# jewettaij/visfd

Hardware: AMD Instinct MI355X
Metric: Mvoxels/s (Gauss+DoG+TV pipeline) on 1024^3 float32; % HBM roofline (higher is better)
Workload: dtype f32

## Files before the change

include/visfd_hip.h:

```cpp
#ifndef VISFD_HIP_H
#define VISFD_HIP_H

#include <stddef.h>
#include <stdint.h>

#ifdef __cplusplus
extern "C" {
#endif

#define VISFD_HIP_OK 0
#define VISFD_HIP_EINVAL 1
#define VISFD_HIP_EDEVICE 2
#define VISFD_HIP_ENOMEM 3
#define VISFD_HIP_ECAPACITY 4

#define VISFD_HIP_INCREASING_EIVALS 0
#define VISFD_HIP_DECREASING_EIVALS 1

typedef struct visfd_hip_ctx visfd_hip_ctx;

int visfd_hip_create(int device, void* stream, visfd_hip_ctx** out);
int visfd_hip_destroy(visfd_hip_ctx* ctx);
int visfd_hip_synchronize(visfd_hip_ctx* ctx);
void* visfd_hip_get_stream(visfd_hip_ctx* ctx);
// ... 503 lines not shown
                                   int64_t nvox, int round, uint32_t prefix,
                                   uint64_t* hist_host , uint64_t* n_unmasked_host);
int visfd_hip_select_histogram_todev(visfd_hip_ctx*, const float* saliency, const float* mask, int64_t nvox, int round,
                                     uint32_t prefix, uint64_t* hist_dev );
int visfd_hip_apply_threshold_dev(visfd_hip_ctx*, float* saliency, int64_t nvox, float threshold);

int visfd_hip_tv_dense_stick(visfd_hip_ctx*, const float* saliency, const float* direction,
                             float* tensor, const float* mask_src, const float* mask_dst,
                             int64_t nx, int64_t ny, int64_t nz, float sigma_tv, int exponent,
                             float cutoff_ratio, int detect_curves);
int visfd_hip_tv_dense_stick_dev(visfd_hip_ctx*, const float* saliency, const float* direction,
                                 float* tensor, const float* mask_src, const float* mask_dst,
                                 int64_t nx, int64_t ny, int64_t nz, float sigma_tv, int exponent,
                                 float cutoff_ratio, int detect_curves);
int visfd_hip_tv_dense_stick_slab_dev(visfd_hip_ctx*, const float* saliency, const float* direction,
                                      float* tensor, const float* mask_src, const float* mask_dst,
                                      int64_t nx, int64_t ny, int64_t nz_local, int64_t z_out0,
                                      int64_t z_out1, float sigma_tv, int exponent,
                                      float cutoff_ratio, int detect_curves);
int visfd_hip_tv_weight_sum(visfd_hip_ctx*, const float* saliency, float* den, const float* mask_src, const float* mask_dst,
                            int64_t nx, int64_t ny, int64_t nz, float sigma_tv, float cutoff_ratio);
int visfd_hip_tv_tables(float sigma_tv, float cutoff_ratio, int* halfwidth_out, float* w,
                        float* rhat);

int visfd_hip_tensor_saliency(visfd_hip_ctx*, const float* tensor, const float* mask, int64_t nvox,
                              int eival_order, float* saliency_inout);
int visfd_hip_tensor_saliency_dev(visfd_hip_ctx*, const float* tensor, const float* mask,
                                  int64_t nvox, int eival_order, float* saliency_inout);
int visfd_hip_tensor_saliency_bg_dev(visfd_hip_ctx*, const float* tensor, const float* mask, int64_t nvox, int eival_order,
                                     const float* image, const float* background, float* saliency_inout);

int visfd_hip_membrane_detect(visfd_hip_ctx*, const float* src, const float* mask,
                              int64_t nx, int64_t ny, int64_t nz, float sigma, float truncate_ratio,
                              int eival_order, float best_fraction, float threshold_abs, float sigma_tv,
                              int tv_exponent, float tv_cutoff_ratio, float* saliency_out,
                              float* tensor_out, float* direction_out, float* threshold_out);
int visfd_hip_membrane_detect_dev(visfd_hip_ctx*, const float* src, const float* mask,
                                  int64_t nx, int64_t ny, int64_t nz, float sigma, float truncate_ratio,
                                  int eival_order, float best_fraction, float threshold_abs,
                                  float sigma_tv, int tv_exponent, float tv_cutoff_ratio,
                                  float* saliency_out, float* tensor_out, float* direction_out,
                                  float* threshold_out);
int visfd_hip_membrane_detect_bg(visfd_hip_ctx*, const float* src, const float* mask,
                                 int64_t nx, int64_t ny, int64_t nz, float sigma, float truncate_ratio,
                                 int eival_order, float best_fraction, float threshold_abs, float sigma_tv,
                                 int tv_exponent, float tv_cutoff_ratio, float sigma_background, int normalize_background,
                                 float* saliency_out, float* tensor_out, float* direction_out, float* threshold_out);
int visfd_hip_membrane_detect_bg_dev(visfd_hip_ctx*, const float* src, const float* mask,
                                     int64_t nx, int64_t ny, int64_t nz, float sigma, float truncate_ratio,
                                     int eival_order, float best_fraction, float threshold_abs,
                                     float sigma_tv, int tv_exponent, float tv_cutoff_ratio, float sigma_background,
                                     int normalize_background, float* saliency_out, float* tensor_out, float* direction_out,
                                     float* threshold_out);

int visfd_hip_apply_gauss_slab_dev(visfd_hip_ctx*, const float* src, float* dst,
                                   int64_t nx, int64_t ny, int64_t nz_local, int64_t z_lo,
                                   int64_t nz_global, const float sigma[3], const int halfwidth[3],
                                   int normalize, float* A_out);

typedef struct visfd_hip_slab visfd_hip_slab;
typedef struct visfd_hip_transport {
  int (*sendrecv)(void* user, int peer, const void* sendbuf, void* recvbuf, size_t bytes, void* stream);
  int (*allreduce_sum_u64)(void* user, uint64_t* buf, size_t count, void* stream);
  int (*group_start)(void* user);
  int (*group_end)(void* user);
  void* user;
} visfd_hip_transport;
int visfd_hip_slab_unique_id(void* id_out_128_bytes);
int visfd_hip_slab_rccl_available(void);
int visfd_hip_slab_create_rccl(visfd_hip_ctx*, const void* unique_id_128_bytes , int rank,
                               int world, int64_t nz_global, int ghost, visfd_hip_slab** out);
int visfd_hip_slab_create_custom(visfd_hip_ctx*, const visfd_hip_transport*, int rank, int world, int64_t nz_global,
                                 int ghost, visfd_hip_slab** out);
int visfd_hip_slab_destroy(visfd_hip_slab*);
int visfd_hip_slab_layout(visfd_hip_slab*, int64_t out[7]);
int visfd_hip_slab_selftest(visfd_hip_slab*, int64_t count);
int visfd_hip_slab_set_reserve(visfd_hip_slab*, int reserve_workgroups);
int visfd_hip_slab_exchange_dev(visfd_hip_slab*, float* const* volumes, int nvol, int64_t nx, int64_t ny, int depth);
int visfd_hip_membrane_detect_slab_dev(visfd_hip_slab*, float* src, float* sal, float* dirs, float* tensor, float* scratch,
                                       int64_t nx, int64_t ny, float sigma, float truncate_ratio, int eival_order,
                                       float best_fraction, float sigma_tv, int exponent, float tv_truncate_ratio,
                                       int src_halo_ready, float* threshold_out);
int visfd_hip_membrane_detect_slab(visfd_hip_slab*, const float* src_owned, int64_t nx, int64_t ny, float sigma,
                                   float truncate_ratio, int eival_order, float best_fraction, float sigma_tv, int exponent,
                                   float tv_truncate_ratio, float* sal_owned, float* tensor_owned, float* threshold_out);
int visfd_hip_membrane_detect_slab_bg_dev(visfd_hip_slab*, float* src, float* sal, float* dirs, float* tensor, float* scratch,
                                          float* background, int64_t nx, int64_t ny, float sigma, float truncate_ratio,
                                          int eival_order, float best_fraction, float sigma_tv, int exponent,
                                          float tv_truncate_ratio, float sigma_background, int normalize_background,
                                          int src_halo_ready, float* threshold_out);
int visfd_hip_membrane_detect_slab_bg(visfd_hip_slab*, const float* src_owned, int64_t nx, int64_t ny, float sigma,
                                      float truncate_ratio, int eival_order, float best_fraction, float sigma_tv, int exponent,
                                      float tv_truncate_ratio, float sigma_background, int normalize_background,
                                      float* sal_owned, float* tensor_owned, float* threshold_out);
int visfd_hip_blob_dog_slab_dev(visfd_hip_slab*, float* src, int64_t nx, int64_t ny, const float* blob_sigma, int n_sigma,
                                float delta_sigma_over_sigma, float truncate_ratio, float minima_threshold,
                                float maxima_threshold, int src_halo_ready,
                                visfd_hip_blob* minima, int64_t minima_capacity, int64_t* n_minima,
                                visfd_hip_blob* maxima, int64_t maxima_capacity, int64_t* n_maxima);
int visfd_hip_blob_halo_depth(const float* blob_sigma, int n_sigma, float delta_sigma_over_sigma, float truncate_ratio,
                              int* depth_out);
int visfd_hip_apply_gauss_slab(visfd_hip_slab*, const float* src_owned, int64_t nx, int64_t ny, const float sigma[3],
                               const int halfwidth[3], int normalize, float* dst_owned, float* A_out);
int visfd_hip_blob_dog_slab(visfd_hip_slab*, const float* src_owned, int64_t nx, int64_t ny, const float* blob_sigma, int n_sigma,
                            float delta_sigma_over_sigma, float truncate_ratio, float minima_threshold, float maxima_threshold,
                            visfd_hip_blob* minima, int64_t minima_capacity, int64_t* n_minima,
// ... 39 lines not shown
```

visfd_amd/api.py:

```python
import ctypes as C
import os
import sys

import numpy as np

_HERE = os.path.dirname(os.path.abspath(__file__))
LIB_PATH = os.environ.get("VISFD_HIP_LIB") or os.path.join(_HERE, "libvisfd_hip.so")

INCREASING_EIVALS = 0
DECREASING_EIVALS = 1

MORPH_DILATE, MORPH_ERODE, MORPH_OPEN, MORPH_CLOSE, MORPH_TOP_HAT_WHITE, MORPH_TOP_HAT_BLACK = range(6)
MORPH_PATH_GENERAL, MORPH_PATH_XRUNS, MORPH_PATH_LEVELS = 0, 1, 2
MEDIAN_PATH_GENERAL, MEDIAN_PATH_TILED = 0, 1
FILTER3D_PATH_GENERAL, FILTER3D_PATH_TILED = 0, 1
DISTANCE_PATH_GENERAL, DISTANCE_PATH_TRANSFORM = 0, 1
DISTANCE_MAX_DIM_SUM = 46340

_fp = C.POINTER(C.c_float)
_ip = C.POINTER(C.c_int)
_i64 = C.c_int64
_vp = C.c_void_p


# ... 150 lines not shown
                                     C.c_float, C.c_float, C.c_int, C.POINTER(Blob), _i64, C.POINTER(_i64),
                                     C.POINTER(Blob), _i64, C.POINTER(_i64)]),
    "visfd_hip_blob_dog_dev": (C.c_int, [_vp, _vp, _vp, _i64, _i64, _i64, _fp, C.c_int, _fp, C.c_float, C.c_float,
                                         C.c_float, C.c_float, C.c_int, C.POINTER(Blob), _i64, C.POINTER(_i64),
                                         C.POINTER(Blob), _i64, C.POINTER(_i64)]),
    "visfd_hip_blob_dog_begin_dev": (C.c_int, [_vp, _vp, _vp, _i64, _i64, _i64, _fp, C.c_int, _fp, C.c_float, C.c_float,
                                               C.c_float, C.c_float, C.c_int, C.POINTER(_vp)]),
    "visfd_hip_blob_dog_end": (C.c_int, [_vp, C.POINTER(Blob), _i64, C.POINTER(_i64), C.POINTER(Blob), _i64, C.POINTER(_i64)]),
    "visfd_hip_blob_dog_abort": (None, [_vp]),
    "visfd_hip_blob_jobs_pending": (C.c_int, [_vp]),
    "visfd_hip_debug_poison_workspace": (C.c_int, [_vp]),
    "visfd_hip_blob_diameters_to_sigmas": (C.c_int, [_fp, C.c_int, _fp]),
    "visfd_hip_blob_sigmas_to_diameters": (C.c_int, [_fp, C.c_int, _fp]),
    "visfd_hip_calc_hessian": (C.c_int, [_vp, _vp, _vp, _vp, _vp, _i64, _i64, _i64, C.c_float, C.c_float]),
    "visfd_hip_calc_hessian_dev": (C.c_int, [_vp, _vp, _vp, _vp, _vp, _i64, _i64, _i64, C.c_float, C.c_float]),
    "visfd_hip_diagonalize_flat_sym3": (C.c_int, [_vp, _vp, _vp, _i64, C.c_int]),
    "visfd_hip_diagonalize_flat_sym3_dev": (C.c_int, [_vp, _vp, _vp, _i64, C.c_int]),
    "visfd_hip_hessian_saliency": (C.c_int, [_vp, _vp, _vp, _i64, C.c_int, _vp, _vp]),
    "visfd_hip_hessian_saliency_dev": (C.c_int, [_vp, _vp, _vp, _i64, C.c_int, _vp, _vp]),
    "visfd_hip_ridge_saliency_dev": (C.c_int, [_vp, _vp, _vp, _i64, _i64, _i64, C.c_float, C.c_float, C.c_int,
                                               _vp, _vp]),
    "visfd_hip_ridge_scores_dev": (C.c_int, [_vp, _vp, _vp, _i64, _i64, _i64, C.c_float, C.c_float, C.c_int, _vp, _vp]),
    "visfd_hip_ridge_directions_dev": (C.c_int, [_vp, _vp, _i64, _i64, _i64, C.c_float, C.c_int, _vp, _vp]),
    "visfd_hip_threshold_fraction": (C.c_int, [_vp, _vp, _vp, _i64, C.c_float, _fp]),
    "visfd_hip_threshold_fraction_dev": (C.c_int, [_vp, _vp, _vp, _i64, C.c_float, _fp]),
    "visfd_hip_select_histogram_dev": (C.c_int, [_vp, _vp, _vp, _i64, C.c_int, C.c_uint32,
                                                 C.POINTER(C.c_uint64), C.POINTER(C.c_uint64)]),
    "visfd_hip_select_histogram_todev": (C.c_int, [_vp, _vp, _vp, _i64, C.c_int, C.c_uint32, _vp]),
    "visfd_hip_get_stream": (_vp, [_vp]),
    "visfd_hip_apply_threshold_dev": (C.c_int, [_vp, _vp, _i64, C.c_float]),
    "visfd_hip_tv_dense_stick": (C.c_int, [_vp, _vp, _vp, _vp, _vp, _vp, _i64, _i64, _i64, C.c_float, C.c_int,
                                           C.c_float, C.c_int]),
    "visfd_hip_tv_dense_stick_dev": (C.c_int, [_vp, _vp, _vp, _vp, _vp, _vp, _i64, _i64, _i64, C.c_float, C.c_int,
                                               C.c_float, C.c_int]),
    "visfd_hip_tv_dense_stick_slab_dev": (C.c_int, [_vp, _vp, _vp, _vp, _vp, _vp, _i64, _i64, _i64, _i64, _i64,
                                                    C.c_float, C.c_int, C.c_float, C.c_int]),
    "visfd_hip_tv_tables": (C.c_int, [C.c_float, C.c_float, _ip, _fp, _fp]),
    "visfd_hip_tv_weight_sum": (C.c_int, [_vp, _vp, _vp, _vp, _vp, _i64, _i64, _i64, C.c_float, C.c_float]),
    "visfd_hip_membrane_detect": (C.c_int, [_vp, _vp, _vp, _i64, _i64, _i64, C.c_float, C.c_float, C.c_int, C.c_float,
                                            C.c_float, C.c_float, C.c_int, C.c_float, _vp, _vp, _vp, _fp]),
    "visfd_hip_membrane_detect_dev": (C.c_int, [_vp, _vp, _vp, _i64, _i64, _i64, C.c_float, C.c_float, C.c_int,
                                                C.c_float, C.c_float, C.c_float, C.c_int, C.c_float, _vp, _vp, _vp,
                                                _fp]),
    "visfd_hip_tensor_saliency": (C.c_int, [_vp, _vp, _vp, _i64, C.c_int, _vp]),
    "visfd_hip_tensor_saliency_dev": (C.c_int, [_vp, _vp, _vp, _i64, C.c_int, _vp]),
    "visfd_hip_peak_background_dev": (C.c_int, [_vp, _vp, _vp, _i64, _i64, _i64, C.c_float, C.c_float, C.c_int, _vp]),
    "visfd_hip_ridge_scores_bg_dev": (C.c_int, [_vp, _vp, _vp, _i64, _i64, _i64, C.c_float, C.c_float, C.c_int, _vp, _vp, _vp]),
    "visfd_hip_tensor_saliency_bg_dev": (C.c_int, [_vp, _vp, _vp, _i64, C.c_int, _vp, _vp, _vp]),
    "visfd_hip_membrane_detect_bg": (C.c_int, [_vp, _vp, _vp, _i64, _i64, _i64, C.c_float, C.c_float, C.c_int, C.c_float,
                                               C.c_float, C.c_float, C.c_int, C.c_float, C.c_float, C.c_int, _vp, _vp, _vp, _fp]),
    "visfd_hip_membrane_detect_bg_dev": (C.c_int, [_vp, _vp, _vp, _i64, _i64, _i64, C.c_float, C.c_float, C.c_int,
                                                   C.c_float, C.c_float, C.c_float, C.c_int, C.c_float, C.c_float, C.c_int,
                                                   _vp, _vp, _vp, _fp]),
    "visfd_hip_membrane_detect_slab_bg_dev": (C.c_int, [_vp, _vp, _vp, _vp, _vp, _vp, _vp, _i64, _i64, C.c_float, C.c_float, C.c_int,
                                                        C.c_float, C.c_float, C.c_int, C.c_float, C.c_float, C.c_int, C.c_int, _fp]),
    "visfd_hip_membrane_detect_slab_bg": (C.c_int, [_vp, _vp, _i64, _i64, C.c_float, C.c_float, C.c_int, C.c_float, C.c_float,
                                                    C.c_int, C.c_float, C.c_float, C.c_int, _vp, _vp, _fp]),
    "visfd_hip_bin_array3d": (C.c_int, [_vp, _vp, C.POINTER(_i64), _vp, C.POINTER(_i64), _ip]),
    "visfd_hip_bin_array3d_dev": (C.c_int, [_vp, _vp, C.POINTER(_i64), _vp, C.POINTER(_i64), _ip]),
    "visfd_hip_unbin_array3d": (C.c_int, [_vp, _vp, C.POINTER(_i64), _vp, C.POINTER(_i64), _ip]),
    "visfd_hip_unbin_array3d_dev": (C.c_int, [_vp, _vp, C.POINTER(_i64), _vp, C.POINTER(_i64), _ip]),
    "visfd_hip_label_connected": (C.c_int, [_vp, _vp, _vp, _i64, _i64, _i64, C.c_float, _vp, C.c_float, C.c_float, C.c_int,
                                            _vp, C.c_float, C.c_float, C.c_int, C.c_int, _i64, C.c_int, C.c_int, C.c_int,
                                            C.POINTER(_i64), _vp, _vp, _vp, _i64]),
    "visfd_hip_label_connected_ex": (C.c_int, [_vp, _vp, _vp, _i64, _i64, _i64, C.c_float, _vp, C.c_float, C.c_float, C.c_int,
                                               _vp, C.c_float, C.c_float, C.c_int, C.c_int, _i64, C.c_int, C.c_int, C.c_int,
                                               C.POINTER(_i64), _vp, _vp, _vp, _i64, _vp, _vp, _vp, _i64, _vp]),
    "visfd_hip_label_connected_device_seeds": (C.c_int, [_vp, _vp, _vp, _vp, _i64, _i64, _i64, C.c_float, _vp, C.c_float,
                                                         C.c_float, C.c_int, _vp, C.c_float, C.c_float, C.c_int, C.c_int, _i64,
                                                         C.c_int, C.c_int, C.c_int, C.POINTER(_i64), _vp, _vp, _vp, _i64, _vp,
                                                         _vp, _vp, _i64, _vp]),
    "visfd_hip_label_connected_device_seeds_last": (C.c_int, [_vp, _ip, C.POINTER(_i64)]),
    "visfd_hip_label_connected_graph": (C.c_int, [_vp] + _LABEL_CONNECTED_EX),
    "visfd_hip_label_connected_graph_dev": (C.c_int, [_vp] + _LABEL_CONNECTED_EX),
    "visfd_hip_label_connected_graph_host": (C.c_int, list(_LABEL_CONNECTED_EX)),
    "visfd_hip_label_connected_graph_last": (C.c_int, [_vp, _ip, C.POINTER(C.c_uint), C.POINTER(_i64), C.POINTER(_i64)]),
    "visfd_hip_label_connected_graph_last_times": (C.c_int, [_vp, _fp]),
    "visfd_hip_label_connected_graph_last_settled": (C.c_int, [_vp, C.POINTER(C.c_uint)]),
    "visfd_hip_principal_directions_host": (C.c_int, [_vp, _vp, _i64, C.c_int, _vp]),
    "visfd_hip_tensor_saliency_host": (C.c_int, [_vp, _vp, _i64, C.c_int, _vp]),
    "visfd_hip_diagonalize_sym3_f32_host": (C.c_int, [_vp, C.c_int, _vp, _vp]),
    "visfd_hip_diagonalize_flat_sym3_host": (C.c_int, [_vp, _vp, _i64, C.c_int]),
    "visfd_hip_convert_flat_sym2_evects3_host": (C.c_int, [_vp, C.c_int, _vp, _vp]),
    "visfd_hip_surface_points": (C.c_int, [_vp, _vp, _vp, _vp, _i64, _i64, _i64, C.c_int, _fp, C.c_float, C.c_int, C.c_float,
                                           _vp, _vp, _i64, C.POINTER(_i64)]),
    "visfd_hip_surface_points_ctx": (C.c_int, [_vp, _vp, _vp, _vp, _vp, _i64, _i64, _i64, C.c_int, _fp, C.c_float, C.c_int,
                                               C.c_float, _vp, _vp, _i64, C.POINTER(_i64)]),
    "visfd_hip_surface_points_dev": (C.c_int, [_vp, _vp, _vp, _vp, _vp, _i64, _i64, _i64, C.c_int, _fp, C.c_float, C.c_int,
                                               C.c_float, _vp, _vp, _i64, C.POINTER(_i64)]),
    "visfd_hip_surface_points_last": (C.c_int, [_vp, C.POINTER(_i64)]),
    "visfd_hip_surface_points_last_times": (C.c_int, [_vp, _fp]),
    "visfd_hip_sphere_overlap": (C.c_float, [C.c_float, C.c_float, C.c_float]),
    "visfd_hip_sort_blobs": (C.c_int, [_fp, _fp, _fp, _i64, C.c_int, C.c_int, C.POINTER(C.c_uint64)]),
    "visfd_hip_discard_masked_blobs": (C.c_int, [_fp, _fp, _fp, C.POINTER(_i64), _vp, _i64, _i64, _i64]),
    "visfd_hip_discard_overlapping_blobs": (C.c_int, [_fp, _fp, _fp, C.POINTER(_i64), C.c_float, C.c_float,
                                                     C.c_float, C.c_int, C.c_int]),
    "visfd_hip_discard_overlapping_blobs_ctx": (C.c_int, [_vp, _vp, _vp, _vp, C.POINTER(_i64), C.c_float, C.c_float,
                                                         C.c_float, C.c_int, C.c_int]),
    "visfd_hip_discard_overlapping_blobs_dev": (C.c_int, [_vp, _vp, _vp, _vp, C.POINTER(_i64), C.c_float, C.c_float,
                                                         C.c_float, C.c_int, C.c_int]),
    "visfd_hip_discard_overlapping_blobs_last": (C.c_int, [_vp, C.POINTER(_i64)]),
    "visfd_hip_discard_overlapping_blobs_last_times": (C.c_int, [_vp, _fp]),
    "visfd_hip_voxelize_mesh": (C.c_int, _VOXELIZE),
    "visfd_hip_voxelize_mesh_dev": (C.c_int, _VOXELIZE),
    "visfd_hip_voxelize_last": (C.c_int, [_vp, C.POINTER(_i64)]),
    "visfd_hip_voxelize_last_times": (C.c_int, [_vp, _fp]),
# ... 1582 lines not shown
    def dilate_dev(self, src, dst, dxyz, b, mask=None):
        self.morph_table_dev(MORPH_DILATE, src, dst, dxyz, b, mask)

    def erode_dev(self, src, dst, dxyz, b, mask=None):
        self.morph_table_dev(MORPH_ERODE, src, dst, dxyz, b, mask)

    def gauss_slab_dev(self, src, dst, z_lo, nz_global, sigma, hw, normalize=True):
        nz, ny, nx = src.shape
        A = C.c_float()
        self._chk(self._L.visfd_hip_apply_gauss_slab_dev(self._h, _dev(src), _dev(dst), nx, ny, nz, int(z_lo),
                                                         int(nz_global), _f3(sigma), _i3(hw), int(normalize),
                                                         C.byref(A)))
        return A.value

    def log_dev(self, src, dst, sigma, delta, ratio, mask=None):
        nz, ny, nx = src.shape
        self._chk(self._L.visfd_hip_apply_log_dev(self._h, _dev(src), _dev(dst), _dev(mask), nx, ny, nz,
                                                  _f3(sigma), float(delta), float(ratio), None, None))

    def blob_dog_dev(self, src, sigmas, mask=None, aspect=None, delta=0.02, ratio=2.5, minima_threshold=np.inf,
                     maxima_threshold=-np.inf, use_ratios=False, cap=1 << 16):
        return self._blob_call(self._L.visfd_hip_blob_dog_dev, _dev(src), _dev(mask), tuple(src.shape), sigmas,
                               aspect, delta, ratio, minima_threshold, maxima_threshold, use_ratios, cap)

    def calc_hessian_dev(self, src, grad, hess, sigma, ratio, mask=None):
        nz, ny, nx = src.shape
        self._chk(self._L.visfd_hip_calc_hessian_dev(self._h, _dev(src), _dev(grad), _dev(hess), _dev(mask), nx,
                                                     ny, nz, float(sigma), float(ratio)))

    def hessian_saliency_dev(self, hess, sal, dirs, order, mask=None):
        self._chk(self._L.visfd_hip_hessian_saliency_dev(self._h, _dev(hess), _dev(mask), sal.numel(), int(order),
                                                         _dev(sal), _dev(dirs)))

    def ridge_saliency_dev(self, src, sal, dirs, sigma, ratio, order, mask=None):
        nz, ny, nx = src.shape
        self._chk(self._L.visfd_hip_ridge_saliency_dev(self._h, _dev(src), _dev(mask), nx, ny, nz, float(sigma),
                                                       float(ratio), int(order), _dev(sal), _dev(dirs)))

    def ridge_scores_dev(self, src, sal, smoothed, sigma, ratio, order, mask=None, background=None):
        nz, ny, nx = src.shape
        self._chk(self._L.visfd_hip_ridge_scores_bg_dev(self._h, _dev(src), _dev(mask), nx, ny, nz, float(sigma),
                                                        float(ratio), int(order), _dev(background), _dev(sal), _dev(smoothed)))

    def peak_background_dev(self, src, background, sigma_background, ratio, mask=None, normalize=True):
        nz, ny, nx = src.shape
        self._chk(self._L.visfd_hip_peak_background_dev(self._h, _dev(src), _dev(mask), nx, ny, nz, float(sigma_background),
                                                        float(ratio), int(bool(normalize)), _dev(background)))

    def ridge_directions_dev(self, smoothed, sal, dirs, sigma, order):
        nz, ny, nx = smoothed.shape
        self._chk(self._L.visfd_hip_ridge_directions_dev(self._h, _dev(smoothed), nx, ny, nz, float(sigma), int(order),
                                                         _dev(sal), _dev(dirs)))

    def threshold_fraction_dev(self, sal, fraction, mask=None):
        thr = C.c_float()
        self._chk(self._L.visfd_hip_threshold_fraction_dev(self._h, _dev(sal), _dev(mask), sal.numel(),
                                                           float(fraction), C.byref(thr)))
        return thr.value

    def select_histogram_dev(self, sal, pass_, prefix, mask=None):
        hist = np.zeros(2048, np.uint64)
        n = C.c_uint64()
        self._chk(self._L.visfd_hip_select_histogram_dev(self._h, _dev(sal), _dev(mask), sal.numel(), int(pass_),
                                                         int(prefix), hist.ctypes.data_as(C.POINTER(C.c_uint64)),
                                                         C.byref(n)))
        return hist, int(n.value)

    def select_histogram_todev(self, sal, pass_, prefix, hist, mask=None):
        assert hist.is_cuda and hist.numel() == 2048 and hist.element_size() == 8 and hist.is_contiguous()
        self._chk(self._L.visfd_hip_select_histogram_todev(self._h, _dev(sal), _dev(mask), sal.numel(), int(pass_),
                                                           int(prefix), hist.data_ptr()))

    def stream_handle(self):
        return int(self._L.visfd_hip_get_stream(self._h) or 0)

    def apply_threshold_dev(self, sal, thr):
        self._chk(self._L.visfd_hip_apply_threshold_dev(self._h, _dev(sal), sal.numel(), float(thr)))

    def tv_dense_stick_dev(self, sal, dirs, tensor, sigma_tv, exponent=4, cutoff=2.0 ** 0.5, mask_src=None,
                           mask_dst=None, curves=False, z_out=None):
        nz, ny, nx = sal.shape
        z0, z1 = (0, nz) if z_out is None else z_out
        self._chk(self._L.visfd_hip_tv_dense_stick_slab_dev(self._h, _dev(sal), _dev(dirs), _dev(tensor),
                                                            _dev(mask_src), _dev(mask_dst), nx, ny, nz, int(z0),
                                                            int(z1), float(sigma_tv), int(exponent), float(cutoff),
                                                            int(curves)))

    def tensor_saliency_dev(self, tensor, sal, order, mask=None, image=None, background=None):
        self._chk(self._L.visfd_hip_tensor_saliency_bg_dev(self._h, _dev(tensor), _dev(mask), sal.numel(), int(order),
                                                           _dev(image), _dev(background), _dev(sal)))


class Slab:

    def __init__(self, ctx, rank, world, nz_global, ghost, transport="rccl", group=None):
        import torch
        import torch.distributed as dist
        self.ctx, self.rank, self.world = ctx, int(rank), int(world)
        self._L = load_library()
        self._h = _vp()
        self._keep = None
        if transport == "rccl_loopback":
            assert world == 1
            idbuf = (C.c_char * 128)()
            ctx._chk(self._L.visfd_hip_slab_unique_id(C.addressof(idbuf)))
            ctx._chk(self._L.visfd_hip_slab_create_rccl(ctx._h, C.addressof(idbuf), 0, 1, nz_global, ghost, C.byref(self._h)))
# ... 192 lines not shown
```

visfd_amd/build.py:

```python
import concurrent.futures
import os
import subprocess
import sys
import time

HERE = os.path.dirname(os.path.abspath(__file__))
ROOT = os.path.dirname(HERE)
CSRC = os.path.join(HERE, "csrc")
OBJDIR = os.path.join(ROOT, "build", "visfd_hip")
LIB = os.path.join(HERE, "libvisfd_hip.so")

SOURCES = ["host_math.cpp", "blob_post.cpp", "connect.cpp", "watershed_host.cpp", "context.hip", "api.hip", "blob_job.hip", "gauss.hip", "blob.hip", "select.hip", "tv.hip", "resample.hip", "slab.hip", "morph.hip", "morph_levels.hip", "extrema.hip", "filter3d.hip", "draw.hip", "watershed.hip", "median.hip", "intensity.hip", "distance.hip", "find_spheres.hip", "discard_overlap.hip", "connect_seeds.hip", "connect_graph_host.cpp", "connect_graph.hip", "voxelize.hip", "surface_points.hip", "close_surface.hip"]
TV_VARIANT = [("tv_tiled.hip", "tv_tiled", ["-fno-slp-vectorize"]), ("tv_box.hip", "tv_box", ["-fno-slp-vectorize"]),
              ("tv_list.hip", "tv_list", ["-fno-slp-vectorize"]),
              ("ridge.hip", "ridge", [])]
PAIR_FLAGS = ["-fno-slp-vectorize"]
VARIANTS = TV_VARIANT + [("gauss_pair.hip", "gauss_pair", PAIR_FLAGS)] + [("gauss_fused.hip", "gauss_fused_h%d" % h, ["-DVH_FUSED_H=%d" % h, "-fno-slp-vectorize"])
                         for h in range(1, 9)]
HEADERS = ["common.hpp", "exact_div.hpp", "tv_common.hpp", "eigen3.hpp", "union_find.hpp", "tile.hpp", "watershed_host.hpp", "intensity.hpp", "connect_host.hpp", "connect_graph.hpp", os.path.join("..", "..", "include", "visfd_hip.h")]

HIPCC = os.environ.get("HIPCC", "/opt/rocm/bin/hipcc")
FLAGS = ["--offload-arch=gfx950", "-O3", "-std=c++17", "-fPIC", "-ffp-contract=off", "-fno-fast-math",
         "-Wall", "-Wno-unused-function"]


def _mtime(p):
    return os.path.getmtime(p) if os.path.exists(p) else 0.0


def _compile(src, obj, extra=()):
    t0 = time.time()
    cmd = [HIPCC] + FLAGS + list(extra) + ["-x", "hip", "-c", os.path.join(CSRC, src), "-o", obj]
    r = subprocess.run(cmd, capture_output=True, text=True)
    return src, r.returncode, r.stdout + r.stderr, time.time() - t0


def build(force=False, jobs=4, verbose=True):
    os.makedirs(OBJDIR, exist_ok=True)
    newest_header = max(_mtime(os.path.join(CSRC, h)) for h in HEADERS)
    todo, objs = [], []
    units = [(s, os.path.splitext(s)[0], []) for s in SOURCES] + VARIANTS
    flagfile = os.path.join(OBJDIR, "flags.txt")
    flagsig = repr((FLAGS, VARIANTS))
    if not os.path.exists(flagfile) or open(flagfile).read() != flagsig:
        force = True
    for s, stem, extra in units:
        obj = os.path.join(OBJDIR, stem + ".o")
        objs.append(obj)
        if force or _mtime(obj) < max(_mtime(os.path.join(CSRC, s)), newest_header):
            todo.append((s, obj, extra))
    if todo:
        with concurrent.futures.ThreadPoolExecutor(max_workers=jobs) as ex:
            for (src, rc, out, dt), (_, obj, _e) in zip(ex.map(lambda a: _compile(*a), todo), todo):
                if verbose:
                    print("[visfd_amd.build] %-22s %5.1fs %s" % (os.path.basename(obj), dt, "ok" if rc == 0 else "FAILED"))
                if rc != 0:
                    sys.stderr.write(out)
                    raise RuntimeError("hipcc failed on " + src)
                elif out.strip() and verbose:
                    sys.stderr.write(out)
    with open(flagfile, "w") as f:
        f.write(flagsig)
    if todo or not os.path.exists(LIB) or _mtime(LIB) < max(_mtime(o) for o in objs):
        cmd = [HIPCC, "--offload-arch=gfx950", "-shared", "-fPIC", "-o", LIB] + objs
        r = subprocess.run(cmd, capture_output=True, text=True)
        if r.returncode != 0:
            sys.stderr.write(r.stdout + r.stderr)
            raise RuntimeError("link failed")
        if verbose:
            print("[visfd_amd.build] linked", LIB)
    build_cli(verbose)
    return LIB
# ... 28 lines not shown
```

visfd_amd/csrc/api.hip:

```cpp
#include <algorithm>
#include <cmath>
#include <vector>

#include "common.hpp"

namespace vh {

int gauss_dev(visfd_hip_ctx* ctx, const float* src, float* dst, const float* mask, i64 nx, i64 ny, i64 nz,
              const float sigma[3], const int hw[3], bool normalize, const GaussOpts& o) {
  VH_REQUIRE(ctx && src && dst && sigma && hw, "null argument");
  std::vector<float> t[3];
  for (int d = 0; d < 3; d++) {
    VH_REQUIRE(sigma[d] >= 0.0f, "sigma must be non-negative");
    VH_REQUIRE(hw[d] >= 0 && hw[d] <= MAX_HALFWIDTH, "filter halfwidth must be in [0, 64]");
    t[d].resize(2 * hw[d] + 1);
    host_gauss_taps(sigma[d], hw[d], t[d].data());
  }
  return dev_separable3d(ctx, src, dst, mask, nx, ny, nz, t[0].data(), hw[0], t[1].data(), hw[1], t[2].data(), hw[2],
                         normalize, o);
}

static int log_pair_try(visfd_hip_ctx* ctx, const float* src, float* dst, i64 nx, i64 ny, i64 nz, const float sa[3],
                        const float sb[3], const int hw[3], float scale, float* A, float* B) {
  if (!ctx || !src || !dst || !sa || !sb || !hw || ctx->opt.log_pair == 0) return GAUSS_DECLINED;
  LogPairRequest rq = {};
  rq.src = src; rq.dst = dst; rq.nx = nx; rq.ny = ny; rq.nz = nz; rq.scale = scale;
  for (int d = 0; d < 3; d++) {
    if (!(sa[d] >= 0.0f) || !(sb[d] >= 0.0f) || hw[d] < 0 || hw[d] > MAX_HALFWIDTH) return GAUSS_DECLINED;
    rq.a[d].h = rq.b[d].h = hw[d];
    host_gauss_taps(sa[d], hw[d], rq.a[d].t);
    host_gauss_taps(sb[d], hw[d], rq.b[d].t);
  }
  const int rc = log_pair_route(ctx, rq);
  if (rc != VISFD_HIP_OK) return rc;
  if (A) *A = (rq.a[0].t[hw[0]] * rq.a[1].t[hw[1]]) * rq.a[2].t[hw[2]];
  if (B) *B = (rq.b[0].t[hw[0]] * rq.b[1].t[hw[1]]) * rq.b[2].t[hw[2]];
  return VISFD_HIP_OK;
}

static int dog_dev(visfd_hip_ctx* ctx, const float* src, float* dst, const float* mask, i64 nx, i64 ny, i64 nz,
                   const float sa[3], const float sb[3], const int hw[3], float scale, float* A, float* B) {
  if (!mask) {
    const int rc = log_pair_try(ctx, src, dst, nx, ny, nz, sa, sb, hw, scale, A, B);
    if (rc != GAUSS_DECLINED) return rc;
  }
  VH_TRY(gauss_dev(ctx, src, dst, mask, nx, ny, nz, sa, hw, true, {A}));
  return gauss_dev(ctx, src, dst, mask, nx, ny, nz, sb, hw, true, {B, dst, scale});
}

LogPlan plan_log(const float sigma[3], float delta, float ratio) {
  LogPlan p;
  for (int d = 0; d < 3; d++) {
    p.sa[d] = (float)(sigma[d] * (1.0 - 0.5 * delta));
    p.sb[d] = (float)(sigma[d] * (1.0 + 0.5 * delta));
    p.hw[d] = (int)std::floor(ratio * std::fmax(p.sa[d], p.sb[d]));
  }
  p.scale = (float)(1.0 / (delta * delta));
// ... 280 lines not shown
  float *aos, *ph, *dm, *dsal, *pdir;
  VH_TRY(st.up_planar(WS_H2D_0, WS_H2D_2, hess, 6, &ph, &aos));
  VH_TRY(st.up(WS_H2D_1, mask, &dm));
  VH_TRY(st.out(WS_H2D_3, &dsal));
  VH_TRY(st.out(WS_H2D_4, &pdir, 3));
  VH_TRY(dev_hessian_saliency(ctx, ph, dm, nvox, order, dsal, pdir));
  VH_TRY(st.down(sal, dsal));
  return st.down_interleaved(dir, pdir, aos, 3, dm, true);
}

int visfd_hip_ridge_saliency_dev(visfd_hip_ctx* ctx, const float* src, const float* mask, int64_t nx, int64_t ny,
                                 int64_t nz, float sigma, float ratio, int order, float* sal, float* dir) {
  VH_REQUIRE(ctx && src && sal && dir, "null argument");
  VH_REQUIRE(order == 0 || order == 1, "unsupported eigenvalue order");
  VH_HIP(hipSetDevice(ctx->device));
  VH_TRY(check_dims(nx, ny, nz));
  float* S = nullptr;
  VH_TRY(gauss_iso_dev(ctx, src, nullptr, mask, nx, ny, nz, sigma, ratio, true, "filter halfwidth", &S));
  return dev_ridge_saliency_fused(ctx, S, mask, nx, ny, nz, sigma, order, sal, dir);
}

int visfd_hip_ridge_scores_bg_dev(visfd_hip_ctx* ctx, const float* src, const float* mask, int64_t nx, int64_t ny,
                                  int64_t nz, float sigma, float ratio, int order, const float* background, float* sal,
                                  float* smoothed) {
  VH_REQUIRE(ctx && src && sal && smoothed, "null argument");
  VH_REQUIRE(smoothed != src && smoothed != sal, "the smoothed volume needs its own buffer");
  VH_REQUIRE(order == 0 || order == 1, "unsupported eigenvalue order");
  VH_HIP(hipSetDevice(ctx->device));
  VH_TRY(check_dims(nx, ny, nz));
  VH_TRY(gauss_iso_dev(ctx, src, smoothed, mask, nx, ny, nz, sigma, ratio, true, "filter halfwidth"));
  return dev_ridge_score(ctx, smoothed, mask, nx, ny, nz, sigma, order, sal, background ? src : nullptr, background);
}
int visfd_hip_ridge_scores_dev(visfd_hip_ctx* ctx, const float* src, const float* mask, int64_t nx, int64_t ny,
                               int64_t nz, float sigma, float ratio, int order, float* sal, float* smoothed) {
  return visfd_hip_ridge_scores_bg_dev(ctx, src, mask, nx, ny, nz, sigma, ratio, order, nullptr, sal, smoothed);
}
int visfd_hip_peak_background_dev(visfd_hip_ctx* ctx, const float* src, const float* mask, int64_t nx, int64_t ny,
                                  int64_t nz, float sigma_background, float ratio, int normalize, float* background) {
  VH_REQUIRE(ctx && src && background && background != src, "bad argument");
  VH_REQUIRE(sigma_background > 0.0f, "the background width must be positive");
  VH_HIP(hipSetDevice(ctx->device));
  VH_TRY(check_dims(nx, ny, nz));
  return gauss_iso_dev(ctx, src, background, mask, nx, ny, nz, sigma_background, ratio, normalize != 0,
                       "background filter halfwidth");
}

int visfd_hip_ridge_directions_dev(visfd_hip_ctx* ctx, const float* smoothed, int64_t nx, int64_t ny, int64_t nz,
                                   float sigma, int order, const float* sal, float* dir) {
  VH_REQUIRE(ctx && smoothed && sal && dir, "null argument");
  VH_REQUIRE(order == 0 || order == 1, "unsupported eigenvalue order");
  VH_HIP(hipSetDevice(ctx->device));
  VH_TRY(check_dims(nx, ny, nz));
  return dev_ridge_directions(ctx, smoothed, sal, nx, ny, nz, sigma, order, dir);
}

int visfd_hip_threshold_fraction_dev(visfd_hip_ctx* ctx, float* sal, const float* mask, int64_t nvox,
                                     float fraction, float* thr_out) {
  VH_REQUIRE(ctx && sal && nvox > 0, "bad argument");
  VH_REQUIRE(fraction >= 0.0f && fraction <= 1.0f, "fraction must be in [0,1]");
  VH_HIP(hipSetDevice(ctx->device));
  return dev_threshold_fraction(ctx, sal, mask, nvox, fraction, thr_out);
}

int visfd_hip_threshold_fraction(visfd_hip_ctx* ctx, float* sal, const float* mask, int64_t nvox, float fraction,
                                 float* thr_out) {
  VH_REQUIRE(ctx && sal && nvox > 0, "bad argument");
  VH_REQUIRE(fraction >= 0.0f && fraction <= 1.0f, "fraction must be in [0,1]");
  VH_HIP(hipSetDevice(ctx->device));
  const Stage st = {ctx, (size_t)nvox};
  float *ds, *dm;
  VH_TRY(st.up(WS_H2D_0, sal, &ds));
  VH_TRY(st.up(WS_H2D_1, mask, &dm));
  VH_TRY(dev_threshold_fraction(ctx, ds, dm, nvox, fraction, thr_out));
  return st.down(sal, ds);
}

int visfd_hip_select_histogram_dev(visfd_hip_ctx* ctx, const float* sal, const float* mask, int64_t nvox,
                                   int pass, uint32_t prefix, uint64_t* hist_host, uint64_t* n_unmasked) {
  VH_REQUIRE(ctx && sal && hist_host && nvox > 0, "bad argument");
  VH_REQUIRE(pass >= 0 && pass <= 2, "round must be 0, 1 or 2");
  VH_HIP(hipSetDevice(ctx->device));
  return dev_select_histogram(ctx, sal, mask, nvox, pass, prefix, hist_host, n_unmasked);
}

int visfd_hip_select_histogram_todev(visfd_hip_ctx* ctx, const float* sal, const float* mask, int64_t nvox, int pass,
                                     uint32_t prefix, uint64_t* hist_dev) {
  VH_REQUIRE(ctx && sal && hist_dev && nvox > 0, "bad argument");
  VH_REQUIRE(pass >= 0 && pass <= 2, "round must be 0, 1 or 2");
  VH_HIP(hipSetDevice(ctx->device));
  return dev_select_histogram_todev(ctx, sal, mask, nvox, pass, prefix, hist_dev);
}

int visfd_hip_apply_threshold_dev(visfd_hip_ctx* ctx, float* sal, int64_t nvox, float thr) {
  VH_REQUIRE(ctx && sal && nvox > 0, "bad argument");
  VH_HIP(hipSetDevice(ctx->device));
  return dev_apply_threshold(ctx, sal, nvox, thr);
}

int visfd_hip_bin_array3d_dev(visfd_hip_ctx* ctx, const float* src, const int64_t size_src[3], float* dst,
                              const int64_t size_dst[3], const int* offset) {
  VH_REQUIRE(ctx && src && dst && size_src && size_dst, "null argument");
  VH_HIP(hipSetDevice(ctx->device));
  return dev_bin_array3d(ctx, src, size_src, dst, size_dst, offset);
}

int visfd_hip_unbin_array3d_dev(visfd_hip_ctx* ctx, const float* src, const int64_t size_src[3], float* dst,
// ... 37 lines not shown

int visfd_hip_tv_dense_stick_slab_dev(visfd_hip_ctx* ctx, const float* sal, const float* dir, float* ten,
                                      const float* mask_src, const float* mask_dst, int64_t nx,
                                      int64_t ny, int64_t nz_local, int64_t z_out0, int64_t z_out1,
                                      float sigma_tv, int exponent, float cutoff, int curves) {
  VH_REQUIRE(ctx && sal && dir && ten, "null argument");
  VH_HIP(hipSetDevice(ctx->device));
  return dev_tv_dense_stick(ctx, sal, dir, ten, mask_src, mask_dst, nx, ny, nz_local, z_out0, z_out1,
                            sigma_tv, exponent, cutoff, curves != 0);
}

int visfd_hip_tv_dense_stick_dev(visfd_hip_ctx* ctx, const float* sal, const float* dir, float* ten,
                                 const float* mask_src, const float* mask_dst, int64_t nx, int64_t ny,
                                 int64_t nz, float sigma_tv, int exponent, float cutoff, int curves) {
  return visfd_hip_tv_dense_stick_slab_dev(ctx, sal, dir, ten, mask_src, mask_dst, nx, ny, nz, 0, nz,
                                           sigma_tv, exponent, cutoff, curves);
}

int visfd_hip_tv_dense_stick(visfd_hip_ctx* ctx, const float* sal, const float* dir, float* ten, const float* mask_src,
                             const float* mask_dst, int64_t nx, int64_t ny, int64_t nz, float sigma_tv, int exponent,
                             float cutoff, int curves) {
  VH_REQUIRE(ctx && sal && dir && ten, "null argument");
  VH_HIP(hipSetDevice(ctx->device));
  VH_TRY(check_dims(nx, ny, nz));
  const Stage st = {ctx, (size_t)(nx * ny * nz)};
  float *dsal, *pdir, *pten, *aos6, *dms = nullptr, *dmd = nullptr;
  VH_TRY(st.up(WS_H2D_0, sal, &dsal));
  VH_TRY(st.up_planar(WS_H2D_1, WS_H2D_2, dir, 3, &pdir));
  VH_TRY(st.out(WS_H2D_3, &pten, 6));
  VH_TRY(st.up(WS_H2D_4, mask_src, &dms));
  if (mask_dst == mask_src) dmd = dms;
  else VH_TRY(st.up(WS_A, mask_dst, &dmd));
  VH_TRY(dev_tv_dense_stick(ctx, dsal, pdir, pten, dms, dmd, nx, ny, nz, 0, nz, sigma_tv, exponent, cutoff, curves != 0));
  VH_TRY(st.out(WS_B, &aos6, 6));
  return st.down_interleaved(ten, pten, aos6, 6, dmd, true);
}

int visfd_hip_tv_weight_sum(visfd_hip_ctx* ctx, const float* sal, float* den, const float* mask_src,
                            const float* mask_dst, int64_t nx, int64_t ny, int64_t nz, float sigma_tv, float cutoff) {
  VH_REQUIRE(ctx && sal && den, "null argument");
  VH_HIP(hipSetDevice(ctx->device));
  VH_TRY(check_dims(nx, ny, nz));
  const Stage st = {ctx, (size_t)(nx * ny * nz)};
  float *dsal, *dden, *dms = nullptr, *dmd = nullptr;
  VH_TRY(st.up(WS_H2D_0, sal, &dsal));
  VH_TRY(st.up(WS_H2D_1, den, &dden));
  VH_TRY(st.up(WS_H2D_4, mask_src, &dms));
  if (mask_dst == mask_src) dmd = dms;
  else VH_TRY(st.up(WS_A, mask_dst, &dmd));
  VH_TRY(dev_tv_weight_sum(ctx, dsal, dden, dms, dmd, nx, ny, nz, sigma_tv, cutoff));
  return st.down(den, dden);
}

int visfd_hip_membrane_detect_bg_dev(visfd_hip_ctx* ctx, const float* src, const float* mask, int64_t nx,
                                     int64_t ny, int64_t nz, float sigma, float ratio, int order,
                                     float best_fraction, float threshold_abs, float sigma_tv, int exponent,
                                     float cutoff, float sigma_background, int normalize_background, float* sal, float* ten,
                                     float* dir, float* thr_out) {
  VH_REQUIRE(ctx && src && sal, "null argument");
  VH_REQUIRE(order == 0 || order == 1, "unsupported eigenvalue order");
  VH_REQUIRE(best_fraction <= 1.0f, "fraction must be <= 1");
  VH_HIP(hipSetDevice(ctx->device));
  VH_TRY(check_dims(nx, ny, nz));
  const i64 n = nx * ny * nz;
  float* d = dir;
  if (!d) VH_TRY(ws(ctx, WS_TVAUX, (size_t)(3 * n), &d));
  float* smoothed = nullptr;
  VH_TRY(ws(ctx, WS_D, (size_t)n, &smoothed));
  float* bg = nullptr;
  if (sigma_background > 0.0f) {
    VH_TRY(ws(ctx, WS_C, (size_t)n, &bg));
    VH_TRY(visfd_hip_peak_background_dev(ctx, src, mask, nx, ny, nz, sigma_background, ratio, normalize_background, bg));
  }
  VH_TRY(visfd_hip_ridge_scores_bg_dev(ctx, src, mask, nx, ny, nz, sigma, ratio, order, bg, sal, smoothed));
  float thr = threshold_abs;
  if (best_fraction >= 0.0f) VH_TRY(dev_threshold_fraction(ctx, sal, mask, n, best_fraction, &thr));
  else VH_TRY(dev_apply_threshold(ctx, sal, n, thr));
  if (thr_out) *thr_out = thr;
  if (dir) VH_HIP(hipMemsetAsync(dir, 0, sizeof(float) * 3 * (size_t)n, ctx->stream));
  VH_TRY(dev_ridge_directions(ctx, smoothed, sal, nx, ny, nz, sigma, order, d));
  if (sigma_tv > 0.0f) {
    float* t = ten;
    if (!t) VH_TRY(ws(ctx, WS_B, (size_t)(6 * n), &t));
    VH_TRY(dev_tv_dense_stick(ctx, sal, d, t, mask, mask, nx, ny, nz, 0, nz, sigma_tv, exponent, cutoff, false));
    VH_TRY(dev_tensor_saliency(ctx, t, mask, n, order, sal, bg ? src : nullptr, bg));
  }
  return VISFD_HIP_OK;
}
int visfd_hip_membrane_detect_dev(visfd_hip_ctx* ctx, const float* src, const float* mask, int64_t nx,
                                  int64_t ny, int64_t nz, float sigma, float ratio, int order,
                                  float best_fraction, float threshold_abs, float sigma_tv, int exponent,
                                  float cutoff, float* sal, float* ten, float* dir, float* thr_out) {
  return visfd_hip_membrane_detect_bg_dev(ctx, src, mask, nx, ny, nz, sigma, ratio, order, best_fraction, threshold_abs, sigma_tv,
                                          exponent, cutoff, 0.0f, 1, sal, ten, dir, thr_out);
}

int visfd_hip_membrane_detect_bg(visfd_hip_ctx* ctx, const float* src, const float* mask, int64_t nx, int64_t ny,
                                 int64_t nz, float sigma, float ratio, int order, float best_fraction,
                                 float threshold_abs, float sigma_tv, int exponent, float cutoff,
                                 float sigma_background, int normalize_background, float* sal, float* ten, float* dir,
                                 float* thr_out) {
  VH_REQUIRE(ctx && src && sal, "null argument");
  VH_HIP(hipSetDevice(ctx->device));
  VH_TRY(check_dims(nx, ny, nz));
  const Stage st = {ctx, (size_t)(nx * ny * nz)};
  float *ds, *dm, *dsal, *pdir, *pten = nullptr, *aos = nullptr;
  VH_TRY(st.up(WS_H2D_0, src, &ds));
  VH_TRY(st.up(WS_H2D_1, mask, &dm));
  VH_TRY(st.out(WS_H2D_2, &dsal));
  VH_TRY(st.out(WS_H2D_3, &pdir, 3));
  if (ten && sigma_tv > 0.0f) {
    VH_TRY(st.out(WS_H2D_4, &pten, 6));
    VH_HIP(hipMemsetAsync(pten, 0, sizeof(float) * 6 * st.n, ctx->stream));
  }
  VH_TRY(visfd_hip_membrane_detect_bg_dev(ctx, ds, dm, nx, ny, nz, sigma, ratio, order, best_fraction, threshold_abs, sigma_tv,
                                          exponent, cutoff, sigma_background, normalize_background, dsal, pten, pdir, thr_out));
  VH_TRY(st.down(sal, dsal));
  if ((ten && pten) || dir) VH_TRY(st.out(WS_A, &aos, 6));
  if (ten && pten) VH_TRY(st.down_interleaved(ten, pten, aos, 6, nullptr, false));
  if (dir) VH_TRY(st.down_interleaved(dir, pdir, aos, 3, nullptr, false));
  return VISFD_HIP_OK;
}
int visfd_hip_membrane_detect(visfd_hip_ctx* ctx, const float* src, const float* mask, int64_t nx, int64_t ny,
                              int64_t nz, float sigma, float ratio, int order, float best_fraction,
                              float threshold_abs, float sigma_tv, int exponent, float cutoff, float* sal,
                              float* ten, float* dir, float* thr_out) {
  return visfd_hip_membrane_detect_bg(ctx, src, mask, nx, ny, nz, sigma, ratio, order, best_fraction, threshold_abs, sigma_tv,
                                      exponent, cutoff, 0.0f, 1, sal, ten, dir, thr_out);
}

int visfd_hip_tensor_saliency_bg_dev(visfd_hip_ctx* ctx, const float* ten, const float* mask, int64_t nvox,
                                     int order, const float* image, const float* background, float* sal) {
  VH_REQUIRE(ctx && ten && sal && nvox > 0, "bad argument");
  VH_REQUIRE((image == nullptr) == (background == nullptr), "image and background come as a pair");
  VH_REQUIRE(order == 0 || order == 1, "unsupported eigenvalue order");
  VH_HIP(hipSetDevice(ctx->device));
  return dev_tensor_saliency(ctx, ten, mask, nvox, order, sal, image, background);
}
int visfd_hip_tensor_saliency_dev(visfd_hip_ctx* ctx, const float* ten, const float* mask, int64_t nvox,
                                  int order, float* sal) {
// ... 175 lines not shown
```

visfd_amd/csrc/common.hpp:

```cpp
#pragma once

#include <hip/hip_runtime.h>

#include <cstdint>
#include <cstdio>
#include <cstring>
#include <string>
#include <vector>

#include "../../include/visfd_hip.h"

namespace vh {

typedef int64_t i64;

void set_error(const std::string& msg);
int fail(int code, const std::string& msg);

#define VH_HIP(expr)                                                                         \
  do {                                                                                       \
    hipError_t _e = (expr);                                                                  \
    if (_e != hipSuccess)                                                                    \
      return vh::fail(_e == hipErrorOutOfMemory ? VISFD_HIP_ENOMEM : VISFD_HIP_EDEVICE,      \
                      std::string(#expr) + ": " + hipGetErrorString(_e));                    \
// ... 20 lines not shown
  WS_HIST,
  WS_TVTAB,
  WS_TVAUX,
  WS_TVSCRATCH,
  WS_TVLIST,
  WS_H2D_0, WS_H2D_1, WS_H2D_2, WS_H2D_3, WS_H2D_4,
  WS_MORPH_TAB,
  WS_MORPH_SRC,
  WS_MORPH_TMP,
  WS_EXT_FLAGS,
  WS_EXT_PARENT,
  WS_EXT_COUNT,
  WS_EXT_COUNTERS,
  WS_EXT_LIST,
  WS_EXT_RANKS,
  WS_F3D_TAB,
  WS_DRAW_OWNER,
  WS_DRAW_TAB,
  WS_WSH_KIND,
  WS_WSH_LINK,
  WS_WSH_C,
  WS_WSH_STATE,
  WS_WSH_SEEDS,
  WS_WSH_FLAGS,
  WS_MEDIAN_TAB,
  WS_INTENSITY,
  WS_DIST_DSQ,
  WS_DIST_STACK,
  WS_DIST_POINTS,
  WS_FS_RECORDS,
  WS_FS_QUERIES,
  WS_CG_WORD,
  WS_CG_AUX,
  WS_CG_LIST,
  WS_CG_REC,
  WS_CG_SEEDS,
  WS_CG_CLUSTER,
  WS_CG_COUNTERS,
  WS_CG_SETTLE,
  WS_CG_LINKS,
  WS_OVL_LIST,
  WS_OVL_CELLS,
  WS_OVL_TEMP,
  WS_VOX_TOGGLE,
  WS_VOX_MESH,
  WS_SP_BITS,
  WS_SP_CHUNKS,
  WS_SP_LIST,
  WS_SP_OUT,
  WS_SP_SCRATCH,
  WS_CS_ACC,
  WS_CS_GRID,
  WS_CS_AUX,
  WS_NSLOTS
};

struct BlobJob;

}

struct visfd_hip_options {
  int gauss_3pass = 0;
  int gauss_cfg = 0;
  int gauss_wg_per_cu = 2;
  int log_pair = 1;
  int log_pair_chunk = 0;
  int tv_dense = 0;
  int tv_fma = 0;
  int gauss_fma = 0;
  int eig_f32 = 0;
  int tv_zrun = 0;
  int tv_no_replay = 0;
  int tv_exact_tiled = 0;
  int tv_no_fold = 0;
  int tv_poison = 0;
  int tv_reserve_wg = 0;
  int tv_max_wg = 0;
  int64_t blob_test_cap = 0;
  int morph_general = 0;
  int morph_levels = 1;
  int filter3d_general = 0;
  int median_general = 0;
  int distance_general = 0;
  int discard_overlap_host = 0;
  int discard_overlap_time = 0;
  int discard_overlap_max_rounds = 256;
  int find_spheres_host = 0;
  int watershed_host = 0;
  int stats_blocks = 0;
  int connect_time = 0;
  int connect_settle = 0;
  int draw_time = 0;
  int voxelize_bisect = 0;
  int voxelize_time = 0;
  int surface_steps_cap = 256;
  int surface_points_time = 0;
  int close_surface_rtol_exp = 5;
  int close_surface_max_cycles = 20;
  int close_surface_time = 0;
  int debug = 0;
};

struct visfd_hip_ctx {
  visfd_hip_options opt;
  int device = 0;
  hipStream_t stream = nullptr;
  bool own_stream = false;
  void* slot_ptr[vh::WS_NSLOTS] = {};
  size_t slot_bytes[vh::WS_NSLOTS] = {};
  std::vector<unsigned char> slot_key[vh::WS_NSLOTS];
  int num_cus = 256;
  hipStream_t aux_stream = nullptr;
  int morph_last_path = -1;
  struct {
    int64_t n = 0, ncols = 0;
    float den = 0.0f;
  } f3d;
  int f3d_last_path = -1;
  int median_last_path = -1;
  int distance_last_path = -1;
  int find_spheres_last_path = -1;
  int64_t discard_overlap_last[8] = {-1, 0, 0, 0, 0, 0, 0, 0};
  float discard_overlap_ms[5] = {-1.0f, -1.0f, -1.0f, -1.0f, -1.0f};
  float draw_ms[3] = {-1.0f, -1.0f, -1.0f};
  int64_t voxelize_stats[4] = {-1, -1, -1, -1};
  float voxelize_ms[3] = {-1.0f, -1.0f, -1.0f};
  int64_t surface_points_last[6] = {-1, 0, -1, -1, -1, -1};
  float surface_points_ms[4] = {-1.0f, -1.0f, -1.0f, -1.0f};
  int64_t close_surface_last[6] = {-1, -1, -1, -1, -1, -1};
  double close_surface_values[2] = {0.0, 0.0};
  float close_surface_ms[3] = {-1.0f, -1.0f, -1.0f};
  int64_t wsh_stats[4] = {-1, -1, -1, -1};
  int64_t connect_seeds[2] = {-1, -1};
  int64_t connect_graph[4] = {-1, 0, -1, -1};
  unsigned connect_graph_settled = 0;
  float connect_graph_ms[8] = {-1.0f, -1.0f, -1.0f, -1.0f, -1.0f, -1.0f, -1.0f, -1.0f};
  std::vector<vh::BlobJob*> blob_jobs;
};

namespace vh {

int blob_jobs_drain(visfd_hip_ctx* ctx, const BlobJob* except = nullptr);
void blob_jobs_abort(visfd_hip_ctx* ctx);

int ws_get(visfd_hip_ctx* ctx, Slot s, size_t bytes, void** out);
template <typename T>
inline int ws(visfd_hip_ctx* ctx, Slot s, size_t count, T** out) {
  void* p = nullptr;
  int rc = ws_get(ctx, s, count * sizeof(T), &p);
  *out = static_cast<T*>(p);
  return rc;
}
bool ws_holds(const visfd_hip_ctx* ctx, Slot s, const void* key, size_t key_bytes);
int ws_put(visfd_hip_ctx* ctx, Slot s, const void* key, size_t key_bytes, const void* host, size_t bytes);

inline int check_dims(i64 nx, i64 ny, i64 nz) {
  if (nx <= 0 || ny <= 0 || nz <= 0) return fail(VISFD_HIP_EINVAL, "image dimensions must be positive");
  return VISFD_HIP_OK;
}
inline bool overlap_bytes(const void* a, size_t na, const void* b, size_t nb) {
  const char* p = static_cast<const char*>(a);
  const char* q = static_cast<const char*>(b);
  return p && q && p < q + nb && q < p + na;
}
inline bool overlaps(const float* a, const float* b, i64 n) { return overlap_bytes(a, sizeof(float) * n, b, sizeof(float) * n); }
// ... 91 lines not shown

constexpr int GAUSS_DECLINED = -1;
int dev_norm_lines(visfd_hip_ctx* ctx, float* D, i64 nx, i64 ny, i64 nz, const Taps& tx, const Taps& ty, const Taps& tz);

struct LogPairRequest {
  const float* src;
  float* dst;
  i64 nx, ny, nz;
  Taps a[3], b[3];
  float scale;
  i64 z_lo, nz_global;
};
int log_pair_route(visfd_hip_ctx* ctx, const LogPairRequest& rq);

int gauss_dev(visfd_hip_ctx* ctx, const float* src, float* dst, const float* mask, i64 nx, i64 ny, i64 nz,
              const float sigma[3], const int hw[3], bool normalize, const GaussOpts& o = {});
struct LogPlan {
  float sa[3], sb[3], scale;
  int hw[3];
};
LogPlan plan_log(const float sigma[3], float delta, float ratio);
int log_dev(visfd_hip_ctx* ctx, const float* src, float* dst, const float* mask, i64 nx, i64 ny, i64 nz,
            const float sigma[3], float delta, float ratio, float* A, float* B);
int dev_sub_square(visfd_hip_ctx* ctx, const float* a, const float* b, float* out, i64 n);
int dev_scale_clamp_sqrt(visfd_hip_ctx* ctx, float* a_inout, i64 n, float scale);

struct ScanPending {
  const unsigned long long* counters = nullptr;
  const void* survivors = nullptr;
  size_t cap_idx = 0, cap_out = 0;
};
int blob_scan_launch(visfd_hip_ctx* ctx, const BlobJob* owner, int set, hipEvent_t done, const float* lo, const float* mid,
                     const float* hi, const float* mask, i64 nx, i64 ny, i64 nz, float min_thr, float max_thr,
                     ScanPending* pending);
int blob_scan_collect(visfd_hip_ctx* ctx, const ScanPending& pending, hipEvent_t done, hipStream_t aux, i64 nx, i64 ny,
                      int scale_index,
                      float sigma, std::vector<visfd_hip_blob>* minima, std::vector<visfd_hip_blob>* maxima,
                      bool* overflow);
int dev_blob_scan(visfd_hip_ctx* ctx, const float* lo, const float* mid, const float* hi,
                  const float* mask, i64 nx, i64 ny, i64 nz, int scale_index, float sigma,
                  float min_thr, float max_thr, bool want_min, bool want_max,
                  std::vector<visfd_hip_blob>* minima, std::vector<visfd_hip_blob>* maxima);

int dev_hessian(visfd_hip_ctx* ctx, const float* smoothed, const float* mask, i64 nx, i64 ny, i64 nz,
                float sigma, float* grad_planar, float* hess_planar);
int dev_hessian_saliency(visfd_hip_ctx* ctx, const float* hess_planar, const float* mask, i64 nvox,
                         int order, float* saliency, float* dir_planar);
int dev_ridge_saliency_fused(visfd_hip_ctx* ctx, const float* smoothed, const float* mask, i64 nx,
                             i64 ny, i64 nz, float sigma, int order, float* saliency,
                             float* dir_planar);
int dev_ridge_score(visfd_hip_ctx* ctx, const float* smoothed, const float* mask, i64 nx, i64 ny, i64 nz,
                    float sigma, int order, float* saliency, const float* peak_img = nullptr, const float* peak_bg = nullptr);
int dev_ridge_directions(visfd_hip_ctx* ctx, const float* smoothed, const float* saliency, i64 nx, i64 ny, i64 nz,
                         float sigma, int order, float* dir_planar);
int dev_diagonalize(visfd_hip_ctx* ctx, const float* m6_planar, float* out6_planar, i64 n, int order);
int dev_tensor_saliency(visfd_hip_ctx* ctx, const float* tensor_planar, const float* mask, i64 nvox,
                        int order, float* saliency, const float* peak_img = nullptr, const float* peak_bg = nullptr);

int dev_select_histogram(visfd_hip_ctx* ctx, const float* sal, const float* mask, i64 nvox, int pass,
                         uint32_t prefix, uint64_t* hist_host, uint64_t* n_unmasked_host);
int dev_select_histogram_todev(visfd_hip_ctx* ctx, const float* sal, const float* mask, i64 nvox, int pass, uint32_t prefix,
                               uint64_t* hist_dev);
int dev_apply_threshold(visfd_hip_ctx* ctx, float* sal, i64 nvox, float thr);
int dev_threshold_fraction(visfd_hip_ctx* ctx, float* sal, const float* mask, i64 nvox, float fraction,
                           float* thr_out);

int dev_tv_dense_stick(visfd_hip_ctx* ctx, const float* sal, const float* dir_planar,
                       float* tensor_planar, const float* mask_src, const float* mask_dst, i64 nx,
                       i64 ny, i64 nz, i64 z_out0, i64 z_out1, float sigma_tv, int exponent,
                       float cutoff, bool curves);

int dev_tv_weight_sum(visfd_hip_ctx* ctx, const float* sal, float* den, const float* mask_src, const float* mask_dst, i64 nx,
                      i64 ny, i64 nz, float sigma_tv, float cutoff);

constexpr int MORPH_RUN_MAX_R = 10;
struct MorphElem {
  i64 n = 0;
  int lo[3] = {0, 0, 0}, hi[3] = {0, 0, 0};
  bool flat = true;
  bool runs = false;
  int R = 0;
  signed char run_len[(2 * MORPH_RUN_MAX_R + 1) * (2 * MORPH_RUN_MAX_R + 1)];
};

int dev_morph_table(visfd_hip_ctx* ctx, const float* src, float* dst, const float* mask, i64 nx, i64 ny, i64 nz,
                    const MorphElem& el, bool dilate, int epi, bool nan_masked, int* path);
int dev_nan_masked(visfd_hip_ctx* ctx, const float* src, const float* mask, float* out, i64 n);
int morph_put_table(visfd_hip_ctx* ctx, const int* dxyz, const float* b, i64 n, MorphElem* el);
int morph_run(visfd_hip_ctx* ctx, const float* src, float* dst, const float* mask, i64 nx, i64 ny, i64 nz, int op,
              MorphElem el);

i64 host_flat_ball_dsq_max(float radius);
constexpr float MORPH_LEVELS_R0 = 5.0f;
int morph_levels_try(visfd_hip_ctx* ctx, const float* src, float* dst, const float* mask, i64 nx, i64 ny, i64 nz, int op,
                     float radius, float radius_max, float bmax, bool* taken);
struct LevelsEpilogue {
  float* dst;
  const float* mask;
  int t;
  unsigned near_bits, far_bits;
  int epi, nan_masked;
};
int dev_distance_levels(visfd_hip_ctx* ctx, const float* src, const float* mask, i64 nx, i64 ny, i64 nz, float level,
                        int32_t* dsq, const LevelsEpilogue& e);

struct MedianTab {
  i64 n = 0;
  int lo[3] = {0, 0, 0}, hi[3] = {0, 0, 0};
  int W = 0, H = 0, D = 0;
};
int median_put_table(visfd_hip_ctx* ctx, const int* dxyz, i64 n, MedianTab* mt);
int median_run(visfd_hip_ctx* ctx, const float* src, float* dst, const float* mask, i64 nx, i64 ny, i64 nz,
               const MedianTab& mt);

int dev_distance_sq(visfd_hip_ctx* ctx, const float* src, const float* mask, i64 nx, i64 ny, i64 nz, float lo, float hi,
// ... 89 lines not shown
```

visfd_amd/csrc/context.hip:

```cpp
#include <cctype>
#include <cstdlib>

#include "common.hpp"

namespace vh {

static thread_local std::string g_last_error;
void set_error(const std::string& msg) { g_last_error = msg; }
int fail(int code, const std::string& msg) {
  g_last_error = msg;
  return code;
}

int ws_get(visfd_hip_ctx* ctx, Slot s, size_t bytes, void** out) {
  if (bytes == 0) bytes = 16;
  if (ctx->slot_bytes[s] < bytes) {
    ctx->slot_key[s].clear();
    if (ctx->slot_ptr[s] && (s == WS_CAND || s == WS_SCANCNT)) VH_TRY(blob_jobs_drain(ctx));
    if (ctx->slot_ptr[s]) {
      VH_HIP(hipStreamSynchronize(ctx->stream));
      VH_HIP(hipFree(ctx->slot_ptr[s]));
      ctx->slot_ptr[s] = nullptr;
      ctx->slot_bytes[s] = 0;
    }
    void* p = nullptr;
    hipError_t e = hipMalloc(&p, bytes);
    if (e != hipSuccess)
      return fail(VISFD_HIP_ENOMEM, "hipMalloc of " + std::to_string(bytes) + " bytes failed: " +
                                        hipGetErrorString(e));
    ctx->slot_ptr[s] = p;
    ctx->slot_bytes[s] = bytes;
  }
  *out = ctx->slot_ptr[s];
  return VISFD_HIP_OK;
}

bool ws_holds(const visfd_hip_ctx* ctx, Slot s, const void* key, size_t key_bytes) {
  const std::vector<unsigned char>& k = ctx->slot_key[s];
  return key_bytes > 0 && k.size() == key_bytes && std::memcmp(k.data(), key, key_bytes) == 0;
}

int ws_put(visfd_hip_ctx* ctx, Slot s, const void* key, size_t key_bytes, const void* host, size_t bytes) {
  ctx->slot_key[s].clear();
  VH_HIP(hipStreamSynchronize(ctx->stream));
  void* d = nullptr;
  VH_TRY(ws_get(ctx, s, bytes, &d));
  VH_HIP(hipMemcpyAsync(d, host, bytes, hipMemcpyHostToDevice, ctx->stream));
  VH_HIP(hipStreamSynchronize(ctx->stream));
  const unsigned char* k = static_cast<const unsigned char*>(key);
  ctx->slot_key[s].assign(k, k + key_bytes);
  return VISFD_HIP_OK;
}

namespace {

struct OptionDesc {
  const char* name;
  int visfd_hip_options::*i = nullptr;
  int64_t visfd_hip_options::*l = nullptr;
  OptionDesc(const char* n, int visfd_hip_options::*f) : name(n), i(f) {}
  OptionDesc(const char* n, int64_t visfd_hip_options::*f) : name(n), l(f) {}
};
#define VH_OPT(field) {#field, &visfd_hip_options::field}
const OptionDesc kOptions[] = {
    VH_OPT(gauss_3pass), VH_OPT(gauss_cfg), VH_OPT(gauss_wg_per_cu), VH_OPT(log_pair), VH_OPT(log_pair_chunk),
    VH_OPT(tv_dense), VH_OPT(tv_fma), VH_OPT(gauss_fma), VH_OPT(eig_f32), VH_OPT(tv_zrun), VH_OPT(tv_no_replay),
    VH_OPT(tv_exact_tiled), VH_OPT(tv_no_fold), VH_OPT(tv_poison), VH_OPT(tv_reserve_wg), VH_OPT(tv_max_wg),
    VH_OPT(blob_test_cap), VH_OPT(morph_general), VH_OPT(morph_levels), VH_OPT(filter3d_general), VH_OPT(median_general),
    VH_OPT(distance_general), VH_OPT(discard_overlap_host), VH_OPT(discard_overlap_time),
    VH_OPT(discard_overlap_max_rounds), VH_OPT(find_spheres_host), VH_OPT(watershed_host), VH_OPT(stats_blocks),
    VH_OPT(connect_time), VH_OPT(connect_settle), VH_OPT(draw_time), VH_OPT(voxelize_bisect), VH_OPT(voxelize_time),
    VH_OPT(surface_steps_cap), VH_OPT(surface_points_time), VH_OPT(close_surface_rtol_exp),
    VH_OPT(close_surface_max_cycles), VH_OPT(close_surface_time), VH_OPT(debug),
};
#undef VH_OPT
bool set_option(visfd_hip_options* o, const char* name, int64_t value) {
  for (const OptionDesc& d : kOptions) {
    if (std::strcmp(d.name, name) != 0) continue;
    if (d.i) o->*(d.i) = (int)value; else o->*(d.l) = value;
    return true;
  }
  return false;
}
bool get_option(const visfd_hip_options* o, const char* name, int64_t* value) {
  for (const OptionDesc& d : kOptions) {
    if (std::strcmp(d.name, name) != 0) continue;
    *value = d.i ? (int64_t)(o->*(d.i)) : o->*(d.l);
    return true;
  }
  return false;
}
void options_from_environment(visfd_hip_options* o) {
  for (const OptionDesc& d : kOptions) {
    std::string env = "VISFD_HIP_";
    for (const char* c = d.name; *c; c++) env += (char)std::toupper((unsigned char)*c);
    if (const char* e = std::getenv(env.c_str())) set_option(o, d.name, (int64_t)std::atoll(e));
  }
}

}
}

using namespace vh;

extern "C" {

int visfd_hip_abi_version(void) { return 10; }
const char* visfd_hip_last_error(void) { return g_last_error.c_str(); }

int visfd_hip_create(int device, void* stream, visfd_hip_ctx** out) {
  VH_REQUIRE(out, "null output pointer");
  int count = 0;
  hipError_t e = hipGetDeviceCount(&count);
  if (e != hipSuccess || count <= 0)
    return fail(VISFD_HIP_EDEVICE, "no HIP device available (libvisfd_hip has no CPU fallback)");
  VH_REQUIRE(device >= 0 && device < count, "bad device ordinal");
  VH_HIP(hipSetDevice(device));
  hipDeviceProp_t prop;
// ... 14 lines not shown
    ctx->own_stream = true;
  }
  *out = ctx;
  return VISFD_HIP_OK;
}

int visfd_hip_set_option(visfd_hip_ctx* ctx, const char* name, int64_t value) {
  VH_REQUIRE(ctx && name, "null argument");
  if (!set_option(&ctx->opt, name, value)) return fail(VISFD_HIP_EINVAL, std::string("unknown option: ") + name);
  return VISFD_HIP_OK;
}

int visfd_hip_get_option(visfd_hip_ctx* ctx, const char* name, int64_t* value) {
  VH_REQUIRE(ctx && name && value, "null argument");
  if (!get_option(&ctx->opt, name, value)) return fail(VISFD_HIP_EINVAL, std::string("unknown option: ") + name);
  return VISFD_HIP_OK;
}

int visfd_hip_trim(visfd_hip_ctx* ctx) {
  VH_REQUIRE(ctx, "null context");
  VH_HIP(hipSetDevice(ctx->device));
  VH_TRY(blob_jobs_drain(ctx));
  VH_HIP(hipStreamSynchronize(ctx->stream));
  for (int s = 0; s < WS_NSLOTS; s++) {
    ctx->slot_key[s].clear();
    if (ctx->slot_ptr[s]) VH_HIP(hipFree(ctx->slot_ptr[s]));
    ctx->slot_ptr[s] = nullptr;
    ctx->slot_bytes[s] = 0;
  }
  return VISFD_HIP_OK;
}

int visfd_hip_debug_poison_workspace(visfd_hip_ctx* ctx) {
  VH_REQUIRE(ctx, "null context");
  VH_HIP(hipSetDevice(ctx->device));
  VH_TRY(blob_jobs_drain(ctx));
  VH_HIP(hipStreamSynchronize(ctx->stream));
  for (int s = 0; s < WS_NSLOTS; s++) {
    ctx->slot_key[s].clear();
    if (ctx->slot_ptr[s]) VH_HIP(hipMemsetAsync(ctx->slot_ptr[s], 0xFF, ctx->slot_bytes[s], ctx->stream));
  }
  VH_HIP(hipStreamSynchronize(ctx->stream));
  return VISFD_HIP_OK;
}

int visfd_hip_blob_jobs_pending(visfd_hip_ctx* ctx) { return ctx ? (int)ctx->blob_jobs.size() : 0; }

int visfd_hip_destroy(visfd_hip_ctx* ctx) {
  if (!ctx) return VISFD_HIP_OK;
  (void)hipSetDevice(ctx->device);
  blob_jobs_abort(ctx);
  int rc = visfd_hip_trim(ctx);
  if (ctx->aux_stream) (void)hipStreamDestroy(ctx->aux_stream);
  if (ctx->own_stream) (void)hipStreamDestroy(ctx->stream);
  delete ctx;
  return rc;
}

void* visfd_hip_get_stream(visfd_hip_ctx* ctx) { return ctx ? (void*)ctx->stream : nullptr; }

int visfd_hip_synchronize(visfd_hip_ctx* ctx) {
  VH_REQUIRE(ctx, "null context");
  VH_HIP(hipStreamSynchronize(ctx->stream));
  return VISFD_HIP_OK;
}

int64_t visfd_hip_workspace_bytes(visfd_hip_ctx* ctx) {
  if (!ctx) return 0;
  int64_t t = 0;
  for (int s = 0; s < WS_NSLOTS; s++) t += (int64_t)ctx->slot_bytes[s];
  return t;
}

}
```

visfd_amd/csrc/ridge.hip:

```cpp
#include "common.hpp"
#include "eigen3.hpp"

namespace vh {

namespace {

constexpr int BLOCK = 256;

struct Stencil {
  const float* S;
  i64 c;
  i64 sx, sy, sz;
  __device__ __forceinline__ float at(int dx, int dy, int dz) const {
    return S[c + dx * sx + dy * sy + dz * sz];
  }
};

__device__ __forceinline__ void hessian_at(const Stencil& f, float s2, float h6[6]) {
  const float f0 = f.at(0, 0, 0);
  const float two_f0 = 2 * f0;
  const float hxx = (f.at(1, 0, 0) + f.at(-1, 0, 0)) - two_f0;
  const float hyy = (f.at(0, 1, 0) + f.at(0, -1, 0)) - two_f0;
  const float hzz = (f.at(0, 0, 1) + f.at(0, 0, -1)) - two_f0;
  const float hxy = 0.25f * (((f.at(1, 1, 0) + f.at(-1, -1, 0)) - f.at(1, -1, 0)) - f.at(-1, 1, 0));
// ... 76 lines not shown
  dir[v] = d[0];
  dir[nvox + v] = d[1];
  dir[2 * nvox + v] = d[2];
}

template <bool F32>
__global__ void __launch_bounds__(BLOCK)
ridge_fused_kernel(const float* __restrict__ S, const float* __restrict__ mask, int nx, int ny, int nz,
                   float sigma, int order, float* __restrict__ sal, float* __restrict__ dir) {
  int ix, iy, iz;
  if (!voxel_of_block(nx, ny, ix, iy, iz)) return;
  const i64 nvox = (i64)nx * ny * nz;
  const i64 v = ((i64)iz * ny + iy) * nx + ix;
  if (mask && mask[v] == 0.0f) { sal[v] = 0.0f; return; }
  const Stencil f = clamped_stencil(S, ix, iy, iz, nx, ny, nz);
  float h6[6];
  hessian_at(f, sigma * sigma, h6);
  float s, d[3];
  saliency_dir<F32>(h6, order, s, d);
  sal[v] = s;
  dir[v] = d[0];
  dir[nvox + v] = d[1];
  dir[2 * nvox + v] = d[2];
}

template <bool F32>
__global__ void __launch_bounds__(BLOCK)
ridge_score_kernel(const float* __restrict__ S, const float* __restrict__ mask, int nx, int ny, int nz,
                   float sigma, int order, float* __restrict__ sal,
                   const float* __restrict__ peak_img, const float* __restrict__ peak_bg) {
  int ix, iy, iz;
  if (!voxel_of_block(nx, ny, ix, iy, iz)) return;
  const i64 v = ((i64)iz * ny + iy) * nx + ix;
  if (mask && mask[v] == 0.0f) { sal[v] = 0.0f; return; }
  const Stencil f = clamped_stencil(S, ix, iy, iz, nx, ny, nz);
  float h6[6];
  hessian_at(f, sigma * sigma, h6);
  double lam[3];
  eig::D3 E[3];
  eig::eig_sym3<F32>(h6, order, lam, E, false);
  const double l1 = (float)lam[0], l2 = (float)lam[1];
  double N = l1 * l1 - l2 * l2;
  N *= N;
  float score = (float)N;
  if (peak_img) score *= peak_img[v] - peak_bg[v];
  __builtin_nontemporal_store(score, &sal[v]);
}

constexpr int DIR_PER = 16;
constexpr int DIR_CHUNK = DIR_PER * BLOCK;
template <bool F32>
__global__ void __launch_bounds__(BLOCK)
ridge_directions_kernel(const float* __restrict__ S, const float* __restrict__ sal, int nx, int ny, int nz,
                        float sigma, int order, float* __restrict__ dir) {
  __shared__ unsigned short list[DIR_CHUNK];
  __shared__ int wave_tot[BLOCK / 64];
  const i64 nvox = (i64)nx * ny * nz;
  const i64 base = (i64)blockIdx.x * DIR_CHUNK;
  const int tid = threadIdx.x, lane = tid & 63, wave = tid >> 6;
  unsigned keep = 0u;
  int cnt = 0;
#pragma unroll
  for (int k = 0; k < DIR_PER; k++) {
    const i64 v = base + k * BLOCK + tid;
    const bool kp = v < nvox && sal[v] != 0.0f;
    keep |= (kp ? 1u : 0u) << k;
    cnt += kp ? 1 : 0;
  }
  int incl = cnt;
#pragma unroll
  for (int d = 1; d < 64; d <<= 1) {
    const int o = __shfl_up(incl, d);
    if (lane >= d) incl += o;
  }
  if (lane == 63) wave_tot[wave] = incl;
  __syncthreads();
  int off = incl - cnt, total = 0;
#pragma unroll
  for (int w = 0; w < BLOCK / 64; w++) {
    const int t = wave_tot[w];
    off += (w < wave) ? t : 0;
    total += t;
  }
#pragma unroll
  for (int k = 0; k < DIR_PER; k++)
    if ((keep >> k) & 1u) list[off++] = (unsigned short)(k * BLOCK + tid);
  __syncthreads();
  const i64 plane = (i64)nx * ny;
  for (int i = tid; i < total; i += BLOCK) {
    const i64 v = base + list[i];
    const int iz = (int)(v / plane);
    const i64 r = v - (i64)iz * plane;
    const int iy = (int)(r / nx), ix = (int)(r - (i64)iy * nx);
    const Stencil f = clamped_stencil(S, ix, iy, iz, nx, ny, nz);
    float h6[6];
    hessian_at(f, sigma * sigma, h6);
    float s, d[3];
    saliency_dir<F32>(h6, order, s, d);
    dir[v] = d[0];
    dir[nvox + v] = d[1];
    dir[2 * nvox + v] = d[2];
  }
}

template <bool F32>
__global__ void __launch_bounds__(BLOCK)
diagonalize_kernel(const float* __restrict__ m, float* __restrict__ out, i64 n, int order) {
  const i64 v = (i64)blockIdx.x * BLOCK + threadIdx.x;
  if (v >= n) return;
  float h6[6], d6[6];
#pragma unroll
  for (int c = 0; c < 6; c++) h6[c] = m[c * n + v];
  eig::diagonalize_flat<F32>(h6, order, d6);
#pragma unroll
  for (int c = 0; c < 6; c++) out[c * n + v] = d6[c];
}

template <bool F32>
// ... 54 lines not shown
int linear_grid(i64 n, unsigned* g) {
  const i64 nb = (n + BLOCK - 1) / BLOCK;
  if (nb > 0x7fffffffLL) return fail(VISFD_HIP_EINVAL, "array too large for one launch");
  *g = (unsigned)(nb < 1 ? 1 : nb);
  return VISFD_HIP_OK;
}

}

int dev_hessian(visfd_hip_ctx* ctx, const float* S, const float* mask, i64 nx, i64 ny, i64 nz,
                float sigma, float* grad, float* hess) {
  if (nx < 3 || ny < 3 || nz < 3)
    return fail(VISFD_HIP_EINVAL, "CalcHessian requires an image at least 3 voxels wide in x,y,z");
  unsigned g;
  VH_TRY(voxel_grid(nx, ny, nz, &g));
  hessian_kernel<<<dim3(g), dim3(BLOCK), 0, ctx->stream>>>(S, mask, (int)nx, (int)ny, (int)nz, sigma,
                                                          grad, hess);
  VH_HIP(hipGetLastError());
  return VISFD_HIP_OK;
}

int dev_hessian_saliency(visfd_hip_ctx* ctx, const float* hess, const float* mask, i64 nvox, int order,
                         float* sal, float* dir) {
  unsigned g;
  VH_TRY(linear_grid(nvox, &g));
  VH_EIG_LAUNCH(hessian_saliency_kernel, dim3(g), hess, mask, nvox, order, sal, dir);
  VH_HIP(hipGetLastError());
  return VISFD_HIP_OK;
}

int dev_ridge_saliency_fused(visfd_hip_ctx* ctx, const float* S, const float* mask, i64 nx, i64 ny,
                             i64 nz, float sigma, int order, float* sal, float* dir) {
  if (nx < 3 || ny < 3 || nz < 3)
    return fail(VISFD_HIP_EINVAL, "ridge detection requires an image at least 3 voxels wide in x,y,z");
  unsigned g;
  VH_TRY(voxel_grid(nx, ny, nz, &g));
  VH_EIG_LAUNCH(ridge_fused_kernel, dim3(g), S, mask, (int)nx, (int)ny, (int)nz, sigma, order, sal, dir);
  VH_HIP(hipGetLastError());
  return VISFD_HIP_OK;
}

int dev_ridge_score(visfd_hip_ctx* ctx, const float* S, const float* mask, i64 nx, i64 ny, i64 nz, float sigma,
                    int order, float* sal, const float* peak_img, const float* peak_bg) {
  if (nx < 3 || ny < 3 || nz < 3)
    return fail(VISFD_HIP_EINVAL, "ridge detection requires an image at least 3 voxels wide in x,y,z");
  unsigned g;
  VH_TRY(voxel_grid(nx, ny, nz, &g));
  VH_EIG_LAUNCH(ridge_score_kernel, dim3(g), S, mask, (int)nx, (int)ny, (int)nz, sigma, order, sal, peak_img, peak_bg);
  VH_HIP(hipGetLastError());
  return VISFD_HIP_OK;
}

int dev_ridge_directions(visfd_hip_ctx* ctx, const float* S, const float* sal, i64 nx, i64 ny, i64 nz, float sigma,
                         int order, float* dir) {
  if (nx < 3 || ny < 3 || nz < 3)
    return fail(VISFD_HIP_EINVAL, "ridge detection requires an image at least 3 voxels wide in x,y,z");
  if (nx >= (1LL << 31) || ny >= (1LL << 31) || nz >= (1LL << 31)) return fail(VISFD_HIP_EINVAL, "dimension too large");
  const i64 nb = (nx * ny * nz + DIR_CHUNK - 1) / DIR_CHUNK;
  if (nb > 0x7fffffffLL) return fail(VISFD_HIP_EINVAL, "volume too large for one launch");
  VH_EIG_LAUNCH(ridge_directions_kernel, dim3((unsigned)nb), S, sal, (int)nx, (int)ny, (int)nz, sigma, order, dir);
  VH_HIP(hipGetLastError());
  return VISFD_HIP_OK;
}

int dev_diagonalize(visfd_hip_ctx* ctx, const float* m, float* out, i64 n, int order) {
  unsigned g;
  VH_TRY(linear_grid(n, &g));
  VH_EIG_LAUNCH(diagonalize_kernel, dim3(g), m, out, n, order);
  VH_HIP(hipGetLastError());
  return VISFD_HIP_OK;
}

int dev_tensor_saliency(visfd_hip_ctx* ctx, const float* ten, const float* mask, i64 nvox, int order,
                        float* sal, const float* peak_img, const float* peak_bg) {
  unsigned g;
  VH_TRY(linear_grid(nvox, &g));
  VH_EIG_LAUNCH(tensor_saliency_kernel, dim3(g), ten, mask, nvox, order, sal, peak_img, peak_bg);
  VH_HIP(hipGetLastError());
  return VISFD_HIP_OK;
}

int dev_interleaved_to_planar(visfd_hip_ctx* ctx, const float* aos, float* planar, i64 n, int ch) {
  unsigned g;
  VH_TRY(linear_grid(n * ch, &g));
  aos_to_planar_kernel<<<dim3(g), dim3(BLOCK), 0, ctx->stream>>>(aos, planar, n, ch);
  VH_HIP(hipGetLastError());
  return VISFD_HIP_OK;
}

int dev_planar_to_interleaved(visfd_hip_ctx* ctx, const float* planar, float* aos, i64 n, int ch,
                              const float* mask) {
  unsigned g;
  VH_TRY(linear_grid(n * ch, &g));
  planar_to_aos_kernel<<<dim3(g), dim3(BLOCK), 0, ctx->stream>>>(planar, aos, n, ch, mask);
  VH_HIP(hipGetLastError());
  return VISFD_HIP_OK;
}

}
```

visfd_amd/csrc/select.hip:

```cpp
#include <cmath>
#include <vector>

#include "common.hpp"

namespace vh {

namespace {

constexpr int BLOCK = 256;
constexpr int NBINS = 2048;

__device__ __forceinline__ uint32_t order_key(float f) {
  const uint32_t u = __float_as_uint(f);
  return (u & 0x80000000u) ? ~u : (u | 0x80000000u);
}
inline float key_to_float(uint32_t k) {
  const uint32_t u = (k & 0x80000000u) ? (k & 0x7fffffffu) : ~k;
  float f;
  std::memcpy(&f, &u, 4);
  return f;
}

__global__ void __launch_bounds__(BLOCK)
histogram_kernel(const float* __restrict__ sal, const float* __restrict__ mask, i64 n, int round,
                 uint32_t prefix, unsigned long long* __restrict__ hist) {
  __shared__ unsigned int lh[NBINS];
  for (int i = threadIdx.x; i < NBINS; i += BLOCK) lh[i] = 0;
  __syncthreads();
  const int shift = (round == 0) ? 21 : (round == 1) ? 10 : 0;
  const uint32_t dmask = (round == 2) ? 0x3ffu : 0x7ffu;
  const int pshift = (round == 0) ? 32 : (round == 1) ? 21 : 10;
  auto count = [&](float v) {
    const uint32_t k = order_key(v);
    if (round > 0 && (k >> pshift) != prefix) return;
    atomicAdd(&lh[(k >> shift) & dmask], 1u);
  };
  const i64 step = (i64)gridDim.x * BLOCK;
  const i64 n4 = (!mask && (reinterpret_cast<uintptr_t>(sal) & 15u) == 0) ? (n >> 2) : 0;
  const float4* sal4 = reinterpret_cast<const float4*>(sal);
  i64 j = (i64)blockIdx.x * BLOCK + threadIdx.x;
  for (; j + step < n4; j += 2 * step) {
    const float4 a = sal4[j], b = sal4[j + step];
    count(a.x); count(a.y); count(a.z); count(a.w);
    count(b.x); count(b.y); count(b.z); count(b.w);
  }
  if (j < n4) {
    const float4 a = sal4[j];
    count(a.x); count(a.y); count(a.z); count(a.w);
  }
  for (i64 i = 4 * n4 + (i64)blockIdx.x * BLOCK + threadIdx.x; i < n; i += step) {
    if (mask && mask[i] == 0.0f) continue;
    count(sal[i]);
  }
  __syncthreads();
  for (int i = threadIdx.x; i < NBINS; i += BLOCK) {
    const unsigned int c = lh[i];
    if (c) atomicAdd(&hist[i], (unsigned long long)c);
  }
}

__global__ void __launch_bounds__(BLOCK)
apply_threshold_kernel(float* __restrict__ sal, i64 n, float thr) {
  i64 i = (i64)blockIdx.x * BLOCK + threadIdx.x;
  const i64 step = (i64)gridDim.x * BLOCK;
  for (; i < n; i += step) {
    const float s = sal[i];
    if (s < thr) sal[i] = 0.0f;
  }
}

}

int dev_select_histogram(visfd_hip_ctx* ctx, const float* sal, const float* mask, i64 nvox, int pass,
                         uint32_t prefix, uint64_t* hist_host, uint64_t* n_unmasked_host) {
  unsigned long long* hist = nullptr;
  VH_TRY(ws(ctx, WS_HIST, (size_t)NBINS, &hist));
  hipStream_t st = ctx->stream;
  VH_HIP(hipMemsetAsync(hist, 0, sizeof(unsigned long long) * NBINS, st));
  const unsigned g = grid_for(nvox, BLOCK, (i64)ctx->num_cus * 32);
  histogram_kernel<<<dim3(g), dim3(BLOCK), 0, st>>>(sal, mask, nvox, pass, prefix, hist);
  VH_HIP(hipGetLastError());
  VH_HIP(hipMemcpyAsync(hist_host, hist, sizeof(uint64_t) * NBINS, hipMemcpyDeviceToHost, st));
  VH_HIP(hipStreamSynchronize(st));
  if (n_unmasked_host) {
    uint64_t tot = 0;
    for (int b = 0; b < NBINS; b++) tot += hist_host[b];
    *n_unmasked_host = tot;
  }
  return VISFD_HIP_OK;
}

int dev_select_histogram_todev(visfd_hip_ctx* ctx, const float* sal, const float* mask, i64 nvox, int pass, uint32_t prefix,
                               uint64_t* hist_dev) {
  hipStream_t st = ctx->stream;
  VH_HIP(hipMemsetAsync(hist_dev, 0, sizeof(unsigned long long) * NBINS, st));
  const unsigned g = grid_for(nvox, BLOCK, (i64)ctx->num_cus * 32);
  histogram_kernel<<<dim3(g), dim3(BLOCK), 0, st>>>(sal, mask, nvox, pass, prefix, reinterpret_cast<unsigned long long*>(hist_dev));
  VH_HIP(hipGetLastError());
  return VISFD_HIP_OK;
}

int dev_apply_threshold(visfd_hip_ctx* ctx, float* sal, i64 nvox, float thr) {
  const unsigned g = grid_for(nvox, BLOCK, (i64)ctx->num_cus * 32);
  apply_threshold_kernel<<<dim3(g), dim3(BLOCK), 0, ctx->stream>>>(sal, nvox, thr);
  VH_HIP(hipGetLastError());
  return VISFD_HIP_OK;
}

static int pick_bin_descending(const std::vector<uint64_t>& h, uint64_t* k) {
  uint64_t seen = 0;
  for (int b = NBINS - 1; b >= 0; b--) {
    if (seen + h[b] > *k) { *k -= seen; return b; }
    seen += h[b];
  }
  return -1;
}

int select_pick_digit(const uint64_t* hist, uint64_t* k) {
  return pick_bin_descending(std::vector<uint64_t>(hist, hist + NBINS), k);
}
float select_key_to_float(uint32_t key) { return key_to_float(key); }

int dev_threshold_fraction(visfd_hip_ctx* ctx, float* sal, const float* mask, i64 nvox, float fraction,
                           float* thr_out) {
  std::vector<uint64_t> h(NBINS);
  uint64_t n_unmasked = 0;
  VH_TRY(dev_select_histogram(ctx, sal, mask, nvox, 0, 0, h.data(), &n_unmasked));
  const float prod = (float)n_unmasked * fraction;
  uint64_t k = (uint64_t)std::floor(prod);
  if (n_unmasked == 0 || k >= n_unmasked)
    return fail(VISFD_HIP_EINVAL, "threshold fraction selects no voxel (the reference would read past its array)");
  const int d0 = pick_bin_descending(h, &k);
  if (d0 < 0) return fail(VISFD_HIP_EDEVICE, "radix select: inconsistent histogram");
  VH_TRY(dev_select_histogram(ctx, sal, mask, nvox, 1, (uint32_t)d0, h.data(), nullptr));
  const int d1 = pick_bin_descending(h, &k);
  if (d1 < 0) return fail(VISFD_HIP_EDEVICE, "radix select: inconsistent histogram");
  VH_TRY(dev_select_histogram(ctx, sal, mask, nvox, 2, ((uint32_t)d0 << 11) | (uint32_t)d1, h.data(), nullptr));
  const int d2 = pick_bin_descending(h, &k);
  if (d2 < 0) return fail(VISFD_HIP_EDEVICE, "radix select: inconsistent histogram");
  const float thr = key_to_float(((uint32_t)d0 << 21) | ((uint32_t)d1 << 10) | (uint32_t)d2);
  if (thr_out) *thr_out = thr;
  return dev_apply_threshold(ctx, sal, nvox, thr);
}

}
```

visfd_amd/csrc/tv.hip:

```cpp
#include <vector>

#include "tv_common.hpp"

namespace vh {

namespace {

constexpr int BLOCK = 256;

struct TvParams {
  int nx, ny, nz;
  int z_out0, z_out1;
  int h;
  int exponent;
  int curves;
  int weights_only;
};

__device__ __forceinline__ float decay_of(float ang, int exponent) {
  if (exponent == 2) return ang;
  if (exponent == 4) return ang * ang;
  return (float)pow((double)ang, 0.5 * (double)exponent);
}

// ... 131 lines not shown
  p.nx = (int)rq.nx; p.ny = (int)rq.ny; p.nz = (int)rq.nz;
  p.z_out0 = (int)rq.z_out0; p.z_out1 = (int)rq.z_out1;
  p.h = tab.h; p.exponent = rq.exponent; p.curves = rq.curves ? 1 : 0; p.weights_only = rq.weights_only ? 1 : 0;
  const i64 nb = ((rq.nx + BLOCK - 1) / BLOCK) * rq.ny * (rq.z_out1 - rq.z_out0);
  if (nb > 0x7fffffffLL) return fail(VISFD_HIP_EINVAL, "volume too large for one launch");
  tv_dense_kernel<<<dim3((unsigned)nb), dim3(BLOCK), 0, ctx->stream>>>(rq.sal, rq.dir, rq.out, rq.mask_src, rq.mask_dst,
                                                                       tab.packed, p);
  VH_HIP(hipGetLastError());
  return VISFD_HIP_OK;
}

int tv_dispatch(visfd_hip_ctx* ctx, const TvRequest& rq, float sigma_tv, float cutoff) {
  const int h = host_tv_halfwidth(sigma_tv, cutoff);
  VH_REQUIRE(h >= 0 && h <= 255, "tensor-voting window halfwidth out of range");
  TvTables tab;
  VH_TRY(tv_table_device(ctx, sigma_tv, cutoff, h, &tab));
  TvRoute routes[4];
  const int nroutes = tv_routes(ctx->opt, rq, routes);
  int rc = TV_DECLINED;
  for (int i = 0; i < nroutes && rc == TV_DECLINED; i++) {
    switch (routes[i]) {
      case TvRoute::BoxTol:
      case TvRoute::BoxExact: {
        const bool exact = routes[i] == TvRoute::BoxExact;
        rc = dev_tv_box(ctx, rq.sal, rq.dir, rq.out, rq.mask_src, rq.mask_dst, rq.nx, rq.ny, rq.nz, rq.z_out0, rq.z_out1, h,
                        exact ? tab.box_exact : tab.box_tol, tab.box_tol_sq, rq.exponent, exact);
        break;
      }
      case TvRoute::Tiled:
        rc = dev_tv_tiled(ctx, rq.sal, rq.dir, rq.out, rq.mask_src, rq.mask_dst, rq.nx, rq.ny, rq.nz, rq.z_out0, rq.z_out1, h,
                          tab.padded, rq.exponent, rq.curves, rq.weights_only);
        break;
      case TvRoute::Baseline:
        rc = tv_baseline(ctx, rq, tab);
        break;
    }
  }
  return rc;
}

}

int dev_tv_dense_stick(visfd_hip_ctx* ctx, const float* sal, const float* dir, float* ten,
                       const float* mask_src, const float* mask_dst, i64 nx, i64 ny, i64 nz,
                       i64 z_out0, i64 z_out1, float sigma_tv, int exponent, float cutoff, bool curves) {
  VH_TRY(check_dims(nx, ny, nz));
  VH_TRY(check_dims32(nx, ny, nz));
  VH_REQUIRE(z_out0 >= 0 && z_out1 <= nz && z_out0 <= z_out1, "bad receiver plane range");
  if (z_out0 == z_out1) return VISFD_HIP_OK;
  return tv_dispatch(ctx, {sal, dir, ten, mask_src, mask_dst, nx, ny, nz, z_out0, z_out1, exponent, curves, false}, sigma_tv,
                     cutoff);
}

int dev_tv_weight_sum(visfd_hip_ctx* ctx, const float* sal, float* den, const float* mask_src, const float* mask_dst, i64 nx,
                      i64 ny, i64 nz, float sigma_tv, float cutoff) {
  VH_TRY(check_dims(nx, ny, nz));
  VH_TRY(check_dims32(nx, ny, nz));
  return tv_dispatch(ctx, {sal, nullptr, den, mask_src, mask_dst, nx, ny, nz, 0, nz, 4, false, true}, sigma_tv, cutoff);
}

}
```

visfd_amd/csrc/tv_box.hip:

```cpp
#include <algorithm>
#include <type_traits>
#include <vector>

#include "tv_common.hpp"

namespace vh {

using namespace box_tile;

namespace {

constexpr int NH = TX / 8;
constexpr int NLIST = 2;
constexpr int NSUB = 2;
constexpr int LSLOTS = NT;
constexpr int HCAP = 36;
constexpr int YPAD = 3;

typedef float f4v __attribute__((ext_vector_type(4)));
typedef unsigned u4v __attribute__((ext_vector_type(4)));
typedef unsigned u2v __attribute__((ext_vector_type(2)));

#ifdef VH_TV_STAMPS
__device__ unsigned long long g_box_stamps[8];
// ... 685 lines not shown
          __syncthreads();
          VH_STAMP(4);
          done += NT;
        } while (done < total);
      }

#pragma unroll
      for (int q = 0; q < NPAIR; q++)
#pragma unroll
        for (int pp = 0; pp < NH; pp++) {
          const int rx = x0 + 8 * pp + 4 * sub + lcol, ry = y0 + 4 * wave + lrow, rzl = rz + 2 * q + lpl;
          const bool in = rx < p.nx && ry < p.ny && rzl < z_run1;
          const i64 rc = (i64)rzl * plane + (i64)ry * p.nx + rx;
          const bool live = in && !(mask_dst && mask_dst[in ? rc : 0] == 0.0f);
          if (live) {
#pragma unroll
            for (int k = 0; k < 6; k++) __builtin_nontemporal_store(TT[q][pp][k], &ten[k * nvox + rc]);
          }
        }
    }
  }
#ifdef VH_TV_STAMPS
  VH_STAMP(5);
  if (lane == 0) {
#pragma unroll
    for (int i = 0; i < 6; i++) atomicAdd(&g_box_stamps[i], st_acc[i]);
  }
#endif
#ifdef VH_TV_COUNT
  if (lane == 0) {
    atomicAdd(&g_box_counts[0], (unsigned long long)cnt_tested);
    atomicAdd(&g_box_counts[1], (unsigned long long)cnt_hits);
    atomicAdd(&g_box_counts[2], (unsigned long long)cnt_steps);
  }
#endif
}

__global__ void __launch_bounds__(256) lds_poison_kernel(unsigned* sink) {
  extern __shared__ unsigned pz[];
  for (int i = threadIdx.x; i < 160 * 256; i += 256) pz[i] = 0xffffffffu;
  __syncthreads();
  if (pz[(threadIdx.x * 37) % (160 * 256)] == 1u) sink[0] = 1u;
}

auto box_exact_kernel(int mode) {
  if (mode == 0) return tv_boxx_kernel<0>;
  return tv_boxx_kernel<2>;
}
auto box_tol_kernel(int mode, bool fold) {
  if (mode == 0) return fold ? tv_box_kernel<0, true> : tv_box_kernel<0, false>;
  return fold ? tv_box_kernel<2, true> : tv_box_kernel<2, false>;
}

}

int dev_tv_box(visfd_hip_ctx* ctx, const float* sal, const float* dir, float* ten, const float* mask_src,
               const float* mask_dst, i64 nx, i64 ny, i64 nz, i64 z_out0, i64 z_out1, int h, const float4* dtab_box,
               const float4* dtab_box_sq, int exponent, bool exact) {
  if (exponent != 2 && exponent != 4) return TV_DECLINED;
  if (h < 1 || h > 40) return TV_DECLINED;
  if (nx * ny >= (1LL << 29) || nx > TV_LIST_MAX_NX || ny >= (1 << 24)) return TV_DECLINED;
  hipStream_t st = ctx->stream;
  BoxParams p;
  p.nx = (int)nx; p.ny = (int)ny; p.nz = (int)nz;
  p.z_out0 = (int)z_out0; p.z_out1 = (int)z_out1;
  p.h = h;
  p.rw = TX + 2 * h;
  p.rh = TY + 2 * h;
  if (p.rw > 255 || p.rh > 255) return TV_DECLINED;
  p.sp = tv_box_row(h);
  p.nsl = tv_box_slice(h);
  const size_t slice_bytes = sizeof(float4) * (size_t)p.nsl;
  p.tiles_x = (int)((nx + TX - 1) / TX);
  p.tiles_y = (int)((ny + TY - 1) / TY);
  i64 nblk = 0;
  VH_TRY(tv_plan_units(ctx, 8, p.tiles_x, p.tiles_y, z_out0, z_out1, &p.zrun, &nblk));
  if (nblk == 0) return VISFD_HIP_OK;
  const size_t lds = 2 * slice_bytes + sizeof(unsigned) * (size_t)(2 * h + 4) * NW * (exact ? NPAIR : 1);
  const size_t lds_static = sizeof(float4) * (LSLOTS + 1) + sizeof(uint2) * LSLOTS + sizeof(uint2) * NW * NSUB * 2 * HCAP + 1536;
  static_assert(2 * HCAP == HX, "the two kernels' hit lists take the same LDS");
  if (lds + lds_static > 150 * 1024) return TV_DECLINED;

  unsigned* counter = nullptr;
  VH_TRY(ws(ctx, WS_COUNTER, 16, &counter));
  TvSenderLists L;
  VH_TRY(tv_sender_lists(ctx, sal, dir, mask_src, nx, ny, nz, z_out0, z_out1, h, exact ? 1 : (exponent == 4 ? 0 : 2),
                         exact ? (TVL_NON_FINITE | TVL_WEIGHTED_MASK) : 0u, !exact && !ctx->opt.tv_no_fold, counter, &L));
  p.zl0 = L.zl0; p.nzl = L.nzl;

  size_t wg_per_cu = (160 * 1024) / (lds + lds_static);
  if (wg_per_cu > 3) wg_per_cu = 3;
  if (wg_per_cu < 1) wg_per_cu = 1;
  const i64 ngrid = tv_plan_grid(ctx, wg_per_cu, nblk);
  if (ctx->opt.tv_poison) {
    VH_HIP(hipMemsetAsync(ten, 0xff, sizeof(float) * 6 * (size_t)(nx * ny * nz), st));
    VH_TRY(tv_launch_lds(ctx, lds_poison_kernel, 1024, 256, 160 * 1024, counter + 8));
  }
  const int md = exponent == 4 ? 0 : 2;
  auto kernel = exact ? box_exact_kernel(md) : box_tol_kernel(md, L.folded);
  const float4* const dtab = (!exact && md == 0 && L.folded) ? dtab_box_sq : dtab_box;
  VH_TRY(tv_launch_lds(ctx, kernel, ngrid, NT, lds, ten, mask_dst, dtab, p, counter, (unsigned)nblk, L.ent, L.pos, L.rows));
  VH_HIP(hipGetLastError());
#ifdef VH_TV_COUNT
  {
    unsigned long long c4[8], z4[8] = {};
    VH_HIP(hipStreamSynchronize(st));
    VH_HIP(hipMemcpyFromSymbol(c4, HIP_SYMBOL(g_box_counts), sizeof(c4)));
    fprintf(stderr, "[tv_box counts] list entries tested %.4g  hits (sender, sub-patch) %.4g  vote steps %.4g  -> hits per tested entry %.3f, "
            "stream fill %.3f\n", (double)c4[0], (double)c4[1], (double)c4[2], (double)c4[1] / (double)c4[0], (double)c4[1] / (2.0 * (double)c4[2]));
    VH_HIP(hipMemcpyToSymbol(HIP_SYMBOL(g_box_counts), z4, sizeof(z4)));
  }
#endif
#ifdef VH_TV_STAMPS
  {
    unsigned long long st8[8], z8[8] = {};
    VH_HIP(hipStreamSynchronize(st));
    VH_HIP(hipMemcpyFromSymbol(st8, HIP_SYMBOL(g_box_stamps), sizeof(st8)));
    double tot = 0;
    for (int i = 0; i < 6; i++) tot += (double)st8[i];
    fprintf(stderr, "[tv_box stamps] share of wave time: listing+claim %.3f | fill %.3f | barrier before sweep %.3f | test+vote %.3f | "
            "barrier after sweep %.3f | stores+rest %.3f  (total %.3g ticks over %lld waves)\n", st8[0] / tot, st8[1] / tot,
            st8[2] / tot, st8[3] / tot, st8[4] / tot, st8[5] / tot, tot, (long long)ngrid * NW);
    VH_HIP(hipMemcpyToSymbol(HIP_SYMBOL(g_box_stamps), z8, sizeof(z8)));
  }
#endif
  return VISFD_HIP_OK;
}

}
```

visfd_amd/csrc/tv_common.hpp:

```cpp
#pragma once

#include <algorithm>

#include "common.hpp"

namespace vh {

constexpr int TV_DECLINED = -1;

inline int tv_padded_row(int h) {
  int sp = 2 * h + 1;
  while ((sp & 7) != 4) sp++;
  return sp;
}

inline int tv_box_row(int h) {
  int sp = 2 * h + 1 + 3;
  while ((sp & 7) != 4) sp++;
  return sp;
}
inline int tv_box_slice(int h) { return (2 * h + 1 + 6) * tv_box_row(h) + 8; }

struct TvTableLayout {
  size_t packed, padded, box_tol, box_exact, box_tol_sq;
// ... 26 lines not shown
namespace box_tile {
constexpr int NT = 512;
constexpr int NW = NT / 64;
constexpr int TX = 16, TY = 4 * NW;
}

inline int tv_plan_units(const visfd_hip_ctx* ctx, int default_zrun, int tiles_x, int tiles_y, i64 z_out0, i64 z_out1,
                         int* zrun, i64* nblk) {
  int zr = default_zrun;
  if (ctx->opt.tv_zrun >= 1 && ctx->opt.tv_zrun <= 4096) zr = ctx->opt.tv_zrun;
  if ((i64)zr > z_out1 - z_out0) zr = (int)(z_out1 - z_out0);
  if (zr < 1) zr = 1;
  const i64 nruns = (z_out1 - z_out0 + zr - 1) / zr;
  *zrun = zr;
  *nblk = std::max<i64>((i64)tiles_x * tiles_y * nruns, 0);
  if (*nblk > 0x7fffffffLL) return fail(VISFD_HIP_EINVAL, "volume too large for one launch");
  return VISFD_HIP_OK;
}
inline i64 tv_plan_grid(const visfd_hip_ctx* ctx, size_t wg_per_cu, i64 nblk) {
  i64 ngrid = (i64)ctx->num_cus * (i64)wg_per_cu;
  if (ctx->opt.tv_reserve_wg > 0) ngrid = std::max<i64>(ngrid - ctx->opt.tv_reserve_wg, 1);
  if (ctx->opt.tv_max_wg > 0 && ngrid > ctx->opt.tv_max_wg) ngrid = ctx->opt.tv_max_wg;
  return std::min(ngrid, nblk);
}

template <typename... KArgs, typename... Args>
inline int tv_launch_lds(visfd_hip_ctx* ctx, void (*kernel)(KArgs...), i64 ngrid, int nthreads, size_t lds, Args... args) {
  VH_HIP(hipFuncSetAttribute(reinterpret_cast<const void*>(kernel), hipFuncAttributeMaxDynamicSharedMemorySize, (int)lds));
  kernel<<<dim3((unsigned)ngrid), dim3(nthreads), lds, ctx->stream>>>(args...);
  return VISFD_HIP_OK;
}

int dev_tv_tiled(visfd_hip_ctx* ctx, const float* sal, const float* dir, float* ten, const float* mask_src,
                 const float* mask_dst, i64 nx, i64 ny, i64 nz, i64 z_out0, i64 z_out1, int h, const float4* dtab, int exponent,
                 bool curves, bool weights_only);
int dev_tv_box(visfd_hip_ctx* ctx, const float* sal, const float* dir, float* ten, const float* mask_src, const float* mask_dst,
               i64 nx, i64 ny, i64 nz, i64 z_out0, i64 z_out1, int h, const float4* dtab_box, const float4* dtab_box_sq, int exponent,
               bool exact);


constexpr int TV_LIST_MAX_NX = 16384;
constexpr unsigned TVL_NOT_POSITIVE = 1u;
constexpr unsigned TVL_NON_FINITE = 2u;
constexpr unsigned TVL_WEIGHTED_MASK = 4u;
struct TvSenderLists {
  const float4* ent;
  const unsigned* pos;
  const unsigned* rows;
  unsigned long long total;
  unsigned flags;
  bool folded;
  int zl0, nzl;
};
int tv_sender_lists(visfd_hip_ctx* ctx, const float* sal, const float* dir, const float* mask_src, i64 nx, i64 ny, i64 nz,
                    i64 z_out0, i64 z_out1, int h, int mode, unsigned decline_on, bool may_fold, unsigned* counter,
                    TvSenderLists* out);

}
```

visfd_amd/csrc/tv_list.hip:

```cpp
#include <algorithm>

#include "tv_common.hpp"

namespace vh {

using namespace box_tile;

namespace {

struct ListGeo {
  int nx, ny, nz;
  int zl0, nzl;
  int ntx, h;
};
constexpr int LNT = 256;
constexpr int LWORDS_MAX = TV_LIST_MAX_NX / 32;

__device__ __forceinline__ unsigned popc_range(const unsigned* w, int lo, int hi) {
  unsigned c = 0;
  for (int i = lo >> 5; i <= (hi - 1) >> 5 && lo < hi; i++) {
    unsigned m = w[i];
    if (i == (lo >> 5)) m &= ~0u << (lo & 31);
    if (i == ((hi - 1) >> 5) && (hi & 31)) m &= ~0u >> (32 - (hi & 31));
    c += (unsigned)__builtin_popcount(m);
  }
  return c;
}

template <bool WRITE, int MODE>
__global__ void __launch_bounds__(LNT)
tvl_row_kernel(const float* __restrict__ sal, const float* __restrict__ dir, const float* __restrict__ mask_src, ListGeo g,
               unsigned* __restrict__ rows, float4* __restrict__ ent, unsigned* __restrict__ pos,
               unsigned* __restrict__ neg_flag ,
               int fold ) {
  constexpr int LB = 8;
  __shared__ unsigned bits_all[LNT / 64][LWORDS_MAX + 4];
  __shared__ unsigned base_all[WRITE ? LNT / 64 : 1][WRITE ? LWORDS_MAX * 2 + 4 : 1];
  __shared__ unsigned cum_all[WRITE ? LNT / 64 : 1][WRITE ? LWORDS_MAX / 2 + 4 : 1];
  const int wave = __builtin_amdgcn_readfirstlane((int)threadIdx.x >> 6), lane = threadIdx.x & 63;
  const i64 r = (i64)blockIdx.x * (LNT / 64) + wave;
  if (r >= (i64)g.nzl * g.ny) return;
  unsigned* const bits = bits_all[wave];
  const int y = (int)(r % g.ny), zl = (int)(r / g.ny);
  const i64 plane = (i64)g.nx * g.ny, nvox = plane * g.nz;
  const i64 row = (i64)(g.zl0 + zl) * plane + (i64)y * g.nx;
  const int nchunks = (g.nx + 63) >> 6;
  unsigned* const rrow = rows + ((size_t)zl * (size_t)(g.ny + 1) + (size_t)y) * (size_t)g.ntx;
  if (WRITE) {
    unsigned* const base = base_all[WRITE ? wave : 0];
    for (int tx = lane; tx < g.ntx; tx += 64) base[tx] = rrow[g.ntx + tx];
  }
  unsigned any = 0, total = 0;
  unsigned* const cum = cum_all[WRITE ? wave : 0];
  for (int c0 = 0; c0 < nchunks; c0 += LB) {
    float v[LB], m[LB];
#pragma unroll
    for (int k = 0; k < LB; k++) {
      const int x = 64 * (c0 + k) + lane;
      v[k] = x < g.nx ? sal[row + x] : 0.0f;
      m[k] = (mask_src && x < g.nx) ? mask_src[row + x] : 1.0f;
    }
#pragma unroll
    for (int k = 0; k < LB; k++) {
      if (c0 + k >= nchunks) break;
      const bool f = v[k] != 0.0f && m[k] != 0.0f;
      const unsigned long long bal = __builtin_amdgcn_ballot_w64(f);
      if (lane == 0) {
        bits[2 * (c0 + k)] = (unsigned)bal;
        bits[2 * (c0 + k) + 1] = (unsigned)(bal >> 32);
        if (WRITE) cum[c0 + k] = total;
      }
      any |= (unsigned)bal | (unsigned)(bal >> 32);
      if (WRITE) total += (unsigned)__builtin_popcountll(bal);
      if (!WRITE && f) {
        const float s = mask_src ? v[k] * m[k] : v[k];
        if (!(s > 0.0f)) atomicOr(neg_flag, 1u);
        if (!(__builtin_fabsf(s) <= 3.402823466e38f)) atomicOr(neg_flag, 2u);
        if (mask_src && m[k] != 1.0f) atomicOr(neg_flag, 4u);
      }
    }
  }
  __builtin_amdgcn_wave_barrier();
  asm volatile("s_waitcnt vmcnt(0) lgkmcnt(0)" ::: "memory");
  if (!WRITE) {
    for (int tx = lane; tx < g.ntx; tx += 64)
      rrow[tx] = any ? popc_range(bits, max(TX * tx - g.h, 0), min(TX * tx + TX + g.h, g.nx)) : 0u;
    return;
  }
  if (!any) return;
  const unsigned* const base = base_all[WRITE ? wave : 0];
  for (unsigned j0 = 0; j0 < total; j0 += 64) {
    const unsigned j = j0 + lane;
    if (j >= total) break;
    int lo = 0, hi = nchunks;
    while (hi - lo > 1) {
      const int mid = (lo + hi) >> 1;
      if (cum[mid] <= j) lo = mid; else hi = mid;
    }
    unsigned k = j - cum[lo];
    unsigned w = bits[2 * lo];
    int x = 64 * lo;
    {
      const unsigned t = (unsigned)__builtin_popcount(w);
      if (k >= t) { k -= t; x += 32; w = bits[2 * lo + 1]; }
    }
#pragma unroll
    for (int sft = 16; sft >= 1; sft >>= 1) {
      const unsigned t = (unsigned)__builtin_popcount(w & ((1u << sft) - 1u));
      if (k >= t) { k -= t; x += sft; w >>= sft; }
    }
    float4 q = make_float4(sal[row + x] * (MODE == 0 ? 0.25f : (MODE == 2 ? 0.5f : 1.0f)), dir[row + x], dir[nvox + row + x], dir[2 * nvox + row + x]);
    if (mask_src) q.x = q.x * mask_src[row + x];
    if (fold) {
      const double r2 = sqrt((double)q.x);
      const float a = (float)(MODE == 0 ? cbrt(r2) : sqrt(r2));
      q = make_float4(2.0f * a * a, a * q.y, a * q.z, a * q.w);
    }
    const int t0 = max((x - TX - g.h) / TX + ((x - TX - g.h) >= 0 ? 1 : 0), 0);
    const int t1 = min((x + g.h) / TX, g.ntx - 1);
    for (int tx = t0; tx <= t1; tx++) {
      const int lo_x = TX * tx - g.h, hi_x = min(TX * tx + TX + g.h, g.nx);
      if (x < lo_x || x >= hi_x) continue;
      const unsigned idx = base[tx] + popc_range(bits, x + 1, hi_x);
      ent[idx] = q;
      pos[idx] = (unsigned)(x - lo_x) | ((unsigned)y << 8);
    }
  }
}

__global__ void __launch_bounds__(LNT)
tvl_scan_kernel(ListGeo g, unsigned* __restrict__ rows, unsigned long long* __restrict__ total) {
  const int i = blockIdx.x * LNT + threadIdx.x;
  if (i >= g.nzl * g.ntx) return;
  const int zl = i / g.ntx, tx = i - zl * g.ntx;
  unsigned* const col = rows + (size_t)zl * (size_t)(g.ny + 1) * (size_t)g.ntx + tx;
  unsigned sum = 0;
  for (int y = 0; y < g.ny; y++) sum += col[(size_t)y * g.ntx];
  const unsigned base = (unsigned)atomicAdd(total, (unsigned long long)sum);
  unsigned run = base;
  unsigned prev = col[(size_t)(g.ny - 1) * g.ntx];
  col[(size_t)g.ny * g.ntx] = run;
  for (int y = g.ny - 1; y >= 0; y--) {
    const unsigned c = prev;
    if (y > 0) prev = col[(size_t)(y - 1) * g.ntx];
    run += c;
    col[(size_t)y * g.ntx] = run;
  }
}

}

int tv_sender_lists(visfd_hip_ctx* ctx, const float* sal, const float* dir, const float* mask_src, i64 nx, i64 ny, i64 nz,
                    i64 z_out0, i64 z_out1, int h, int mode, unsigned decline_on, bool may_fold, unsigned* counter,
                    TvSenderLists* out) {
  hipStream_t st = ctx->stream;
  ListGeo g;
  g.nx = (int)nx; g.ny = (int)ny; g.nz = (int)nz; g.h = h; g.ntx = (int)((nx + TX - 1) / TX);
  g.zl0 = (int)std::max<i64>(z_out0 - h, 0);
  g.nzl = (int)(std::min<i64>(z_out1 + h, nz) - g.zl0);
  const size_t nrows = (size_t)g.nzl * (size_t)(ny + 1) * (size_t)g.ntx;
  if ((i64)g.nzl * ny > 0x7fffffffLL) return TV_DECLINED;
  unsigned* rows = nullptr;
  if (ws(ctx, WS_TVLIST, nrows, &rows) != VISFD_HIP_OK) { set_error(""); (void)hipGetLastError(); return TV_DECLINED; }
  unsigned long long* total_dev = reinterpret_cast<unsigned long long*>(counter + 4);
  VH_HIP(hipMemsetAsync(counter, 0, 16 * sizeof(unsigned), st));
  const unsigned row_blocks = (unsigned)(((i64)g.nzl * ny + LNT / 64 - 1) / (LNT / 64));
  const auto row_pass = [&](auto kernel, float4* ent, unsigned* pos, int fold) {
    kernel<<<dim3(row_blocks), dim3(LNT), 0, st>>>(sal, dir, mask_src, g, rows, ent, pos, counter + 6, fold);
  };
  row_pass(mode == 1 ? tvl_row_kernel<false, 1> : mode == 0 ? tvl_row_kernel<false, 0> : tvl_row_kernel<false, 2>, nullptr, nullptr, 0);
  tvl_scan_kernel<<<dim3((unsigned)(((size_t)g.nzl * g.ntx + LNT - 1) / LNT)), dim3(LNT), 0, st>>>(g, rows, total_dev);
  VH_HIP(hipGetLastError());
  unsigned long long tot2[2] = {0, 0};
  VH_HIP(hipMemcpyAsync(tot2, total_dev, sizeof(tot2), hipMemcpyDeviceToHost, st));
  VH_HIP(hipStreamSynchronize(st));
  const unsigned long long total = tot2[0];
  const unsigned flags = (unsigned)tot2[1];
  if (flags & decline_on) return TV_DECLINED;
  if (total >= (1ull << 32) - 2048) return TV_DECLINED;
  const int fold = (may_fold && !(flags & TVL_NOT_POSITIVE)) ? 1 : 0;
  unsigned char* lists = nullptr;
  if (ws(ctx, WS_TVSCRATCH, (size_t)(total + 16) * 20, &lists) != VISFD_HIP_OK) { set_error(""); (void)hipGetLastError(); return TV_DECLINED; }
  float4* const ent = reinterpret_cast<float4*>(lists);
  unsigned* const pos = reinterpret_cast<unsigned*>(lists + (size_t)(total + 16) * 16);
  if (ctx->opt.tv_poison) VH_HIP(hipMemsetAsync(lists, 0xff, (size_t)(total + 16) * 20, st));
  row_pass(mode == 1 ? tvl_row_kernel<true, 1> : mode == 0 ? tvl_row_kernel<true, 0> : tvl_row_kernel<true, 2>, ent, pos, fold);
  VH_HIP(hipGetLastError());
  *out = {ent, pos, rows, total, flags, fold != 0, g.zl0, g.nzl};
  return VISFD_HIP_OK;
}

}
```

visfd_amd/pipeline.py:

```python
import math

import numpy as np

from . import api

TRUNCATE_THRESHOLD = 0.03


def cli_blob_sigmas(width_min, width_max, growth):
    wmin, wmax, g = np.float32(width_min), np.float32(width_max), np.float32(growth)
    N = 1 + int(math.ceil(np.float32(np.log(np.float32(wmax / wmin), dtype=np.float32) / np.log(g, dtype=np.float32))))
    g = np.float32(math.pow(float(np.float32(wmax / wmin)), 1.0 / N))
    d = np.empty(N, np.float32)
    d[0] = np.float32(wmin * np.float32(2.0 * math.sqrt(3.0)))
    for n in range(1, N):
        d[n] = np.float32(d[n - 1] * g)
    return api.diameters_to_sigmas(d)


def intensity_tail(ctx, src, out, mask=None, invert=False, map=api.MAP_NONE, t=(), out_a=0.0, out_b=1.0,
                   masked_value=None, rescale_min_max=None):
    ave = None
    if invert:
        st = ctx.image_stats(out, mask)
# ... 1 lines not shown
            raise ValueError("intensity_tail: the mean of this image depends on the order of summation")
        ave = st["sum"] / st["count"] if st["count"] else float("nan")
    reads_src = map in (api.MAP_STEP, api.MAP_THRESH2, api.MAP_THRESH4, api.MAP_RANGE, api.MAP_GAUSS)
    p = api.intensity(map, t, out_a, out_b, invert_ave=ave, masked_value=masked_value if mask is not None else None,
                      stats_mask=True)
    staged = invert or map != api.MAP_NONE or p.mask_fill
    if rescale_min_max is None:
        if staged:
            ctx.intensity_map(p, out, src if reads_src else None, mask)
        return
    st = ctx.intensity_map(p, out, src if reads_src else None, mask, want_stats=True) if staged else ctx.image_stats(out, mask)
    if st["n_nonfinite"]:
        raise ValueError("intensity_tail: -rescale-min-max of an image with NaN or infinite voxels")
    hi, lo = rescale_min_max
    ctx.intensity_map(api.intensity(rescale01=(st["min"], st["max"], lo, hi)), out)


def gauss(ctx, src, dst, sigma, truncate_threshold=TRUNCATE_THRESHOLD, mask=None, normalize=True, tail=None):
    ratio = api.ratio_from_threshold(truncate_threshold)
    sig = (sigma,) * 3 if np.isscalar(sigma) else tuple(sigma)
    hw = api.gauss_halfwidths(sig, ratio)
    A = ctx.gauss_dev(src, dst, sig, hw, mask, normalize)
    if tail is not None:
        intensity_tail(ctx, src, dst, mask, **tail)
    return A


def blob_detect(ctx, src, sigmas, truncate_threshold=TRUNCATE_THRESHOLD, delta=0.02, mask=None,
                minima_threshold=np.inf, maxima_threshold=-np.inf, use_ratios=False, cap=1 << 22):
    ratio = api.ratio_from_threshold(truncate_threshold)
    return ctx.blob_dog_dev(src, sigmas, mask, None, delta, ratio, minima_threshold, maxima_threshold,
                            use_ratios, cap)


def blob_detect_begin(ctx, src, sigmas, truncate_threshold=TRUNCATE_THRESHOLD, delta=0.02, mask=None,
                      minima_threshold=np.inf, maxima_threshold=-np.inf, use_ratios=False):
    ratio = api.ratio_from_threshold(truncate_threshold)
    return ctx.blob_dog_begin_dev(src, sigmas, mask, None, delta, ratio, minima_threshold, maxima_threshold, use_ratios)


def blob_detect_end(ctx, job, cap=1 << 22):
    return ctx.blob_dog_end(job, cap)


def membrane_detect(ctx, src, sal, dirs, tensor, sigma, tv_sigma_ratio, tv_exponent=4, best_fraction=0.05,
                    truncate_threshold=TRUNCATE_THRESHOLD, tv_truncate_ratio=math.sqrt(2.0), minima=True,
                    mask=None, scratch=None, sigma_background=0.0, background=None, tail=None):
    order = api.DECREASING_EIVALS if minima else api.INCREASING_EIVALS
    ratio = api.ratio_from_threshold(truncate_threshold)
    smoothed = scratch if scratch is not None else src.new_empty(src.shape)
    bg = None
    if sigma_background > 0:
        bg = background if background is not None else src.new_empty(src.shape)
        ctx.peak_background_dev(src, bg, sigma_background, ratio, mask)
    ctx.ridge_scores_dev(src, sal, smoothed, sigma, ratio, order, mask, bg)
    thr = ctx.threshold_fraction_dev(sal, best_fraction, mask)
    ctx.ridge_directions_dev(smoothed, sal, dirs, sigma, order)
    sigma_tv = float(np.float32(tv_sigma_ratio) * np.float32(sigma))
    ctx.tv_dense_stick_dev(sal, dirs, tensor, sigma_tv, tv_exponent, tv_truncate_ratio, mask, mask)
    ctx.tensor_saliency_dev(tensor, sal, order, mask, src if bg is not None else None, bg)
    if tail is not None:
        if tail.get("map", api.MAP_NONE) not in (api.MAP_NONE, api.MAP_RESCALE):
            raise ValueError("membrane_detect: the threshold maps read the input image; only MAP_RESCALE acts on the saliency")
        intensity_tail(ctx, src, sal, mask, **tail)
    return thr
```

Measured before the change: 2771.

## Queue membrane stage on device with async threshold readback and thresholded TV lists

Adds a membrane_stage path that computes the best-fraction threshold on device and leaves it there. The TV sender-list counting kernels and ridge-direction kernels read that device threshold directly, and the host readback of threshold and list totals happens asynchronously while the direction kernel runs. This removes host synchronisations between the select, direction and TV stages. The cost is more code complexity and a fallback to the dense path when the lists decline the volume.

Measured after the change: 2800 (median of 6 runs). 1.1% higher.

```diff
diff --git a/include/visfd_hip.h b/include/visfd_hip.h
--- a/include/visfd_hip.h
+++ b/include/visfd_hip.h
@@ -579,6 +579,17 @@
                                      float sigma_tv, int tv_exponent, float tv_cutoff_ratio, float sigma_background,
                                      int normalize_background, float* saliency_out, float* tensor_out, float* direction_out,
                                      float* threshold_out);
+int visfd_hip_membrane_stage_dev(visfd_hip_ctx*, const float* src, const float* mask, int64_t nx, int64_t ny, int64_t nz,
+                                 float sigma, float truncate_ratio, int eival_order, float best_fraction, float sigma_tv,
+                                 int tv_exponent, float tv_cutoff_ratio, float sigma_background, int normalize_background,
+                                 float* background, float* scratch, float* saliency_out, float* direction_out,
+                                 float* tensor_out, float* threshold_out);
+int visfd_hip_debug_ridge_directions_thr_dev(visfd_hip_ctx*, const float* smoothed, int64_t nx, int64_t ny, int64_t nz,
+                                             float sigma, int eival_order, const float* saliency, const float* thr_dev,
+                                             float* direction_out);
+int visfd_hip_debug_tv_lists_dev(visfd_hip_ctx*, const float* saliency, const float* direction, const float* thr_dev, int64_t nx,
+                                 int64_t ny, int64_t nz, int h, int mode, int fold, uint32_t* rows, int64_t rows_cap, float* entries,
+                                 uint32_t* positions, int64_t entries_cap, int64_t* nrows, int64_t* total, uint32_t* flags);
 
 int visfd_hip_apply_gauss_slab_dev(visfd_hip_ctx*, const float* src, float* dst,
                                    int64_t nx, int64_t ny, int64_t nz_local, int64_t z_lo,
diff --git a/visfd_amd/api.py b/visfd_amd/api.py
--- a/visfd_amd/api.py
+++ b/visfd_amd/api.py
@@ -226,6 +226,11 @@
     "visfd_hip_membrane_detect_bg_dev": (C.c_int, [_vp, _vp, _vp, _i64, _i64, _i64, C.c_float, C.c_float, C.c_int,
                                                    C.c_float, C.c_float, C.c_float, C.c_int, C.c_float, C.c_float, C.c_int,
                                                    _vp, _vp, _vp, _fp]),
+    "visfd_hip_membrane_stage_dev": (C.c_int, [_vp, _vp, _vp, _i64, _i64, _i64, C.c_float, C.c_float, C.c_int, C.c_float,
+                                               C.c_float, C.c_int, C.c_float, C.c_float, C.c_int, _vp, _vp, _vp, _vp, _vp, _fp]),
+    "visfd_hip_debug_ridge_directions_thr_dev": (C.c_int, [_vp, _vp, _i64, _i64, _i64, C.c_float, C.c_int, _vp, _vp, _vp]),
+    "visfd_hip_debug_tv_lists_dev": (C.c_int, [_vp, _vp, _vp, _vp, _i64, _i64, _i64, C.c_int, C.c_int, C.c_int, _vp, _i64, _vp,
+                                               _vp, _i64, C.POINTER(_i64), C.POINTER(_i64), C.POINTER(C.c_uint32)]),
     "visfd_hip_membrane_detect_slab_bg_dev": (C.c_int, [_vp, _vp, _vp, _vp, _vp, _vp, _vp, _i64, _i64, C.c_float, C.c_float, C.c_int,
                                                         C.c_float, C.c_float, C.c_int, C.c_float, C.c_float, C.c_int, C.c_int, _fp]),
     "visfd_hip_membrane_detect_slab_bg": (C.c_int, [_vp, _vp, _i64, _i64, C.c_float, C.c_float, C.c_int, C.c_float, C.c_float,
@@ -1914,6 +1919,38 @@
         self._chk(self._L.visfd_hip_ridge_directions_dev(self._h, _dev(smoothed), nx, ny, nz, float(sigma), int(order),
                                                          _dev(sal), _dev(dirs)))
 
+    def membrane_stage_dev(self, src, sal, dirs, tensor, scratch, sigma, ratio, order, best_fraction, sigma_tv, exponent=4,
+                           cutoff=2.0 ** 0.5, mask=None, sigma_background=0.0, background=None, normalize_background=True):
+        nz, ny, nx = src.shape
+        thr = C.c_float()
+        self._chk(self._L.visfd_hip_membrane_stage_dev(
+            self._h, _dev(src), _dev(mask), nx, ny, nz, float(sigma), float(ratio), int(order), float(best_fraction),
+            float(sigma_tv), int(exponent), float(cutoff), float(sigma_background), int(bool(normalize_background)),
+            _dev(background), _dev(scratch), _dev(sal), _dev(dirs), _dev(tensor), C.byref(thr)))
+        return thr.value
+
+    def debug_ridge_directions_thr_dev(self, smoothed, sal, dirs, sigma, order, thr_dev=None):
+        nz, ny, nx = smoothed.shape
+        self._chk(self._L.visfd_hip_debug_ridge_directions_thr_dev(self._h, _dev(smoothed), nx, ny, nz, float(sigma), int(order),
+                                                                   _dev(sal), _dev(thr_dev), _dev(dirs)))
+
+    def debug_tv_lists_dev(self, sal, dirs, h, mode=0, fold=False, thr_dev=None):
+        nz, ny, nx = sal.shape
+        ntx = (nx + 15) // 16
+        nrows, total, flags = _i64(), _i64(), C.c_uint32()
+        rows = np.empty((nz, ny + 1, ntx), np.uint32)
+        ent, pos = np.empty((0, 4), np.float32), np.empty(0, np.uint32)
+        for _ in range(2):
+            self._chk(self._L.visfd_hip_debug_tv_lists_dev(
+                self._h, _dev(sal), _dev(dirs), _dev(thr_dev), nx, ny, nz, int(h), int(mode), int(bool(fold)),
+                rows.ctypes.data, rows.size, ent.ctypes.data, pos.ctypes.data, pos.size, C.byref(nrows), C.byref(total),
+                C.byref(flags)))
+            assert nrows.value == rows.size
+            if total.value <= pos.size:
+                break
+            ent, pos = np.empty((total.value, 4), np.float32), np.empty(total.value, np.uint32)
+        return rows, ent[:total.value], pos[:total.value], int(flags.value)
+
     def threshold_fraction_dev(self, sal, fraction, mask=None):
         thr = C.c_float()
         self._chk(self._L.visfd_hip_threshold_fraction_dev(self._h, _dev(sal), _dev(mask), sal.numel(),
diff --git a/visfd_amd/build.py b/visfd_amd/build.py
--- a/visfd_amd/build.py
+++ b/visfd_amd/build.py
@@ -17,7 +17,7 @@
 PAIR_FLAGS = ["-fno-slp-vectorize"]
 VARIANTS = TV_VARIANT + [("gauss_pair.hip", "gauss_pair", PAIR_FLAGS)] + [("gauss_fused.hip", "gauss_fused_h%d" % h, ["-DVH_FUSED_H=%d" % h, "-fno-slp-vectorize"])
                          for h in range(1, 9)]
-HEADERS = ["common.hpp", "exact_div.hpp", "tv_common.hpp", "eigen3.hpp", "union_find.hpp", "tile.hpp", "watershed_host.hpp", "intensity.hpp", "connect_host.hpp", "connect_graph.hpp", os.path.join("..", "..", "include", "visfd_hip.h")]
+HEADERS = ["common.hpp", "exact_div.hpp", "tv_common.hpp", "select_pick.hpp", "eigen3.hpp", "union_find.hpp", "tile.hpp", "watershed_host.hpp", "intensity.hpp", "connect_host.hpp", "connect_graph.hpp", os.path.join("..", "..", "include", "visfd_hip.h")]
 
 HIPCC = os.environ.get("HIPCC", "/opt/rocm/bin/hipcc")
 FLAGS = ["--offload-arch=gfx950", "-O3", "-std=c++17", "-fPIC", "-ffp-contract=off", "-fno-fast-math",
diff --git a/visfd_amd/csrc/api.hip b/visfd_amd/csrc/api.hip
--- a/visfd_amd/csrc/api.hip
+++ b/visfd_amd/csrc/api.hip
@@ -3,6 +3,7 @@
 #include <vector>
 
 #include "common.hpp"
+#include "tv_common.hpp"
 
 namespace vh {
 
@@ -389,6 +390,49 @@
   VH_HIP(hipSetDevice(ctx->device));
   VH_TRY(check_dims(nx, ny, nz));
   return dev_ridge_directions(ctx, smoothed, sal, nx, ny, nz, sigma, order, dir);
+}
+
+int visfd_hip_debug_ridge_directions_thr_dev(visfd_hip_ctx* ctx, const float* smoothed, int64_t nx, int64_t ny, int64_t nz,
+                                             float sigma, int order, const float* sal, const float* thr_dev, float* dir) {
+  VH_REQUIRE(ctx && smoothed && sal && dir, "null argument");
+  VH_REQUIRE(order == 0 || order == 1, "unsupported eigenvalue order");
+  VH_HIP(hipSetDevice(ctx->device));
+  VH_TRY(check_dims(nx, ny, nz));
+  return dev_ridge_directions(ctx, smoothed, sal, nx, ny, nz, sigma, order, dir, thr_dev);
+}
+int visfd_hip_debug_tv_lists_dev(visfd_hip_ctx* ctx, const float* sal, const float* dir, const float* thr_dev, int64_t nx,
+                                 int64_t ny, int64_t nz, int h, int mode, int fold, uint32_t* rows, int64_t rows_cap, float* ent,
+                                 uint32_t* pos, int64_t ent_cap, int64_t* nrows, int64_t* total, uint32_t* flags) {
+  VH_REQUIRE(ctx && sal && dir && nrows && total && flags, "null argument");
+  VH_REQUIRE(h >= 1 && h <= 40 && mode >= 0 && mode <= 2, "bad list parameters");
+  VH_HIP(hipSetDevice(ctx->device));
+  VH_TRY(check_dims(nx, ny, nz));
+  VH_TRY(check_dims32(nx, ny, nz));
+  VH_REQUIRE(nx <= TV_LIST_MAX_NX && ny < (1 << 24), "volume too wide for the lists");
+  unsigned* counter = nullptr;
+  VH_TRY(ws(ctx, WS_COUNTER, 16, &counter));
+  TvListPlan plan;
+  int rc = tv_list_count(ctx, sal, thr_dev, nullptr, nx, ny, nz, 0, nz, h, mode, counter,
+                         reinterpret_cast<unsigned long long*>(counter + 4), counter + 6, &plan);
+  VH_REQUIRE(rc != TV_DECLINED, "the lists declined the volume");
+  VH_TRY(rc);
+  unsigned long long tot2[2] = {0, 0};
+  VH_HIP(hipMemcpyAsync(tot2, counter + 4, sizeof(tot2), hipMemcpyDeviceToHost, ctx->stream));
+  VH_HIP(hipStreamSynchronize(ctx->stream));
+  TvSenderLists L;
+  rc = tv_list_write(ctx, plan, sal, dir, nullptr, tot2[0], (unsigned)tot2[1], 0u, fold != 0, &L);
+  VH_REQUIRE(rc != TV_DECLINED, "the lists declined the volume");
+  VH_TRY(rc);
+  *nrows = (int64_t)plan.g.nzl * (int64_t)(ny + 1) * (int64_t)plan.g.ntx;
+  *total = (int64_t)L.total;
+  *flags = L.flags;
+  if (rows && rows_cap >= *nrows) VH_HIP(hipMemcpyAsync(rows, L.rows, sizeof(uint32_t) * (size_t)*nrows, hipMemcpyDeviceToHost, ctx->stream));
+  if (ent && pos && ent_cap >= *total && *total > 0) {
+    VH_HIP(hipMemcpyAsync(ent, L.ent, sizeof(float) * 4 * (size_t)*total, hipMemcpyDeviceToHost, ctx->stream));
+    VH_HIP(hipMemcpyAsync(pos, L.pos, sizeof(uint32_t) * (size_t)*total, hipMemcpyDeviceToHost, ctx->stream));
+  }
+  VH_HIP(hipStreamSynchronize(ctx->stream));
+  return VISFD_HIP_OK;
 }
 
 int visfd_hip_threshold_fraction_dev(visfd_hip_ctx* ctx, float* sal, const float* mask, int64_t nvox,
@@ -532,6 +576,67 @@
   return st.down(den, dden);
 }
 
+static int membrane_queued(visfd_hip_ctx* ctx, i64 nx, i64 ny, i64 nz, float sigma, int order, float best_fraction, float sigma_tv,
+                           int exponent, float cutoff, const float* smoothed, float* sal, float* ten, float* dir, bool zero_dir,
+                           const float* peak_img, const float* peak_bg, float* thr_out) {
+  hipStream_t st = ctx->stream;
+  const i64 n = nx * ny * nz;
+  VH_TRY(select_rank_check((uint64_t)n, best_fraction));
+  if (!ctx->stage_pinned) VH_HIP(hipHostMalloc(&ctx->stage_pinned, sizeof(StageReadback)));
+  if (!ctx->stage_event) VH_HIP(hipEventCreateWithFlags(&ctx->stage_event, hipEventDisableTiming));
+  StageReadback* block = nullptr;
+  VH_TRY(ws(ctx, WS_SELECT, 1, &block));
+  VH_HIP(hipMemsetAsync(block, 0, sizeof(*block), st));
+  VH_TRY(dev_select_queue(ctx, sal, nullptr, n, best_fraction, &block->sel));
+  const float* const thr_dev = &block->sel.thr;
+  TvStagePlan plan;
+  VH_TRY(dev_tv_stage_count(ctx, sal, thr_dev, nullptr, nx, ny, nz, sigma_tv, exponent, cutoff, &block->list_total,
+                            &block->list_flags, &plan));
+  const StageReadback* const got = static_cast<const StageReadback*>(ctx->stage_pinned);
+  VH_HIP(hipMemcpyAsync(ctx->stage_pinned, block, sizeof(*block), hipMemcpyDeviceToHost, st));
+  VH_HIP(hipEventRecord(ctx->stage_event, st));
+  if (zero_dir) VH_HIP(hipMemsetAsync(dir, 0, sizeof(float) * 3 * (size_t)n, st));
+  VH_TRY(dev_ridge_directions(ctx, smoothed, sal, nx, ny, nz, sigma, order, dir, thr_dev));
+  VH_HIP(hipEventSynchronize(ctx->stage_event));
+  float thr = 0.0f;
+  VH_TRY(select_result(got->sel, &thr));
+  if (thr_out) *thr_out = thr;
+  int rc = dev_tv_stage_vote(ctx, plan, got->list_total, got->list_flags, sal, dir, ten, nullptr, nx, ny, nz, exponent);
+  if (rc == TV_DECLINED) {
+    VH_TRY(dev_apply_threshold(ctx, sal, n, thr));
+    rc = dev_tv_dense_stick(ctx, sal, dir, ten, nullptr, nullptr, nx, ny, nz, 0, nz, sigma_tv, exponent, cutoff, false);
+  }
+  VH_TRY(rc);
+  return dev_tensor_saliency(ctx, ten, nullptr, n, order, sal, peak_img, peak_bg);
+}
+
+static int membrane_stage(visfd_hip_ctx* ctx, const float* src, const float* mask, i64 nx, i64 ny, i64 nz, float sigma, float ratio,
+                          int order, float best_fraction, float threshold_abs, float sigma_tv, int exponent, float cutoff,
+                          float sigma_background, int normalize_background, float* bg, float* smoothed, float* sal, float* ten,
+                          float* dir, bool zero_dir, float* thr_out) {
+  const i64 n = nx * ny * nz;
+  if (sigma_background > 0.0f)
+    VH_TRY(visfd_hip_peak_background_dev(ctx, src, mask, nx, ny, nz, sigma_background, ratio, normalize_background, bg));
+  else bg = nullptr;
+  VH_TRY(visfd_hip_ridge_scores_bg_dev(ctx, src, mask, nx, ny, nz, sigma, ratio, order, bg, sal, smoothed));
+  if (ctx->opt.membrane_queue && sigma_tv > 0.0f && best_fraction >= 0.0f && !mask) {
+    const int rc = membrane_queued(ctx, nx, ny, nz, sigma, order, best_fraction, sigma_tv, exponent, cutoff, smoothed, sal, ten, dir,
+                                   zero_dir, bg ? src : nullptr, bg, thr_out);
+    if (rc != TV_DECLINED) return rc;
+  }
+  float thr = threshold_abs;
+  if (best_fraction >= 0.0f) VH_TRY(dev_threshold_fraction(ctx, sal, mask, n, best_fraction, &thr));
+  else VH_TRY(dev_apply_threshold(ctx, sal, n, thr));
+  if (thr_out) *thr_out = thr;
+  if (zero_dir) VH_HIP(hipMemsetAsync(dir, 0, sizeof(float) * 3 * (size_t)n, ctx->stream));
+  VH_TRY(dev_ridge_directions(ctx, smoothed, sal, nx, ny, nz, sigma, order, dir));
+  if (sigma_tv > 0.0f) {
+    VH_TRY(dev_tv_dense_stick(ctx, sal, dir, ten, mask, mask, nx, ny, nz, 0, nz, sigma_tv, exponent, cutoff, false));
+    VH_TRY(dev_tensor_saliency(ctx, ten, mask, n, order, sal, bg ? src : nullptr, bg));
+  }
+  return VISFD_HIP_OK;
+}
+
 int visfd_hip_membrane_detect_bg_dev(visfd_hip_ctx* ctx, const float* src, const float* mask, int64_t nx,
                                      int64_t ny, int64_t nz, float sigma, float ratio, int order,
                                      float best_fraction, float threshold_abs, float sigma_tv, int exponent,
@@ -545,27 +650,26 @@
   const i64 n = nx * ny * nz;
   float* d = dir;
   if (!d) VH_TRY(ws(ctx, WS_TVAUX, (size_t)(3 * n), &d));
-  float* smoothed = nullptr;
+  float *smoothed = nullptr, *bg = nullptr, *t = ten;
   VH_TRY(ws(ctx, WS_D, (size_t)n, &smoothed));
-  float* bg = nullptr;
-  if (sigma_background > 0.0f) {
-    VH_TRY(ws(ctx, WS_C, (size_t)n, &bg));
-    VH_TRY(visfd_hip_peak_background_dev(ctx, src, mask, nx, ny, nz, sigma_background, ratio, normalize_background, bg));
-  }
-  VH_TRY(visfd_hip_ridge_scores_bg_dev(ctx, src, mask, nx, ny, nz, sigma, ratio, order, bg, sal, smoothed));
-  float thr = threshold_abs;
-  if (best_fraction >= 0.0f) VH_TRY(dev_threshold_fraction(ctx, sal, mask, n, best_fraction, &thr));
-  else VH_TRY(dev_apply_threshold(ctx, sal, n, thr));
-  if (thr_out) *thr_out = thr;
-  if (dir) VH_HIP(hipMemsetAsync(dir, 0, sizeof(float) * 3 * (size_t)n, ctx->stream));
-  VH_TRY(dev_ridge_directions(ctx, smoothed, sal, nx, ny, nz, sigma, order, d));
-  if (sigma_tv > 0.0f) {
-    float* t = ten;
-    if (!t) VH_TRY(ws(ctx, WS_B, (size_t)(6 * n), &t));
-    VH_TRY(dev_tv_dense_stick(ctx, sal, d, t, mask, mask, nx, ny, nz, 0, nz, sigma_tv, exponent, cutoff, false));
-    VH_TRY(dev_tensor_saliency(ctx, t, mask, n, order, sal, bg ? src : nullptr, bg));
-  }
-  return VISFD_HIP_OK;
+  if (sigma_background > 0.0f) VH_TRY(ws(ctx, WS_C, (size_t)n, &bg));
+  if (!t && sigma_tv > 0.0f) VH_TRY(ws(ctx, WS_B, (size_t)(6 * n), &t));
+  return membrane_stage(ctx, src, mask, nx, ny, nz, sigma, ratio, order, best_fraction, threshold_abs, sigma_tv, exponent, cutoff,
+                        sigma_background, normalize_background, bg, smoothed, sal, t, d, dir != nullptr, thr_out);
+}
+int visfd_hip_membrane_stage_dev(visfd_hip_ctx* ctx, const float* src, const float* mask, int64_t nx, int64_t ny, int64_t nz,
+                                 float sigma, float ratio, int order, float best_fraction, float sigma_tv, int exponent,
+                                 float cutoff, float sigma_background, int normalize_background, float* background,
+                                 float* scratch, float* sal, float* dir, float* ten, float* thr_out) {
+  VH_REQUIRE(ctx && src && scratch && sal && dir && ten, "null argument");
+  VH_REQUIRE(order == 0 || order == 1, "unsupported eigenvalue order");
+  VH_REQUIRE(best_fraction >= 0.0f && best_fraction <= 1.0f, "fraction must be in [0,1]");
+  VH_REQUIRE(sigma_tv > 0.0f, "the voting width must be positive");
+  VH_REQUIRE(!(sigma_background > 0.0f) || background, "the background needs a volume");
+  VH_HIP(hipSetDevice(ctx->device));
+  VH_TRY(check_dims(nx, ny, nz));
+  return membrane_stage(ctx, src, mask, nx, ny, nz, sigma, ratio, order, best_fraction, 0.0f, sigma_tv, exponent, cutoff,
+                        sigma_background, normalize_background, background, scratch, sal, ten, dir, false, thr_out);
 }
 int visfd_hip_membrane_detect_dev(visfd_hip_ctx* ctx, const float* src, const float* mask, int64_t nx,
                                   int64_t ny, int64_t nz, float sigma, float ratio, int order,
diff --git a/visfd_amd/csrc/common.hpp b/visfd_amd/csrc/common.hpp
--- a/visfd_amd/csrc/common.hpp
+++ b/visfd_amd/csrc/common.hpp
@@ -96,6 +96,7 @@
   WS_CS_ACC,
   WS_CS_GRID,
   WS_CS_AUX,
+  WS_SELECT,
   WS_NSLOTS
 };
 
@@ -109,6 +110,7 @@
   int gauss_wg_per_cu = 2;
   int log_pair = 1;
   int log_pair_chunk = 0;
+  int membrane_queue = 1;
   int tv_dense = 0;
   int tv_fma = 0;
   int gauss_fma = 0;
@@ -155,6 +157,8 @@
   std::vector<unsigned char> slot_key[vh::WS_NSLOTS];
   int num_cus = 256;
   hipStream_t aux_stream = nullptr;
+  void* stage_pinned = nullptr;
+  hipEvent_t stage_event = nullptr;
   int morph_last_path = -1;
   struct {
     int64_t n = 0, ncols = 0;
@@ -352,7 +356,7 @@
 int dev_ridge_score(visfd_hip_ctx* ctx, const float* smoothed, const float* mask, i64 nx, i64 ny, i64 nz,
                     float sigma, int order, float* saliency, const float* peak_img = nullptr, const float* peak_bg = nullptr);
 int dev_ridge_directions(visfd_hip_ctx* ctx, const float* smoothed, const float* saliency, i64 nx, i64 ny, i64 nz,
-                         float sigma, int order, float* dir_planar);
+                         float sigma, int order, float* dir_planar, const float* thr_dev = nullptr);
 int dev_diagonalize(visfd_hip_ctx* ctx, const float* m6_planar, float* out6_planar, i64 n, int order);
 int dev_tensor_saliency(visfd_hip_ctx* ctx, const float* tensor_planar, const float* mask, i64 nvox,
                         int order, float* saliency, const float* peak_img = nullptr, const float* peak_bg = nullptr);
@@ -361,6 +365,23 @@
                          uint32_t prefix, uint64_t* hist_host, uint64_t* n_unmasked_host);
 int dev_select_histogram_todev(visfd_hip_ctx* ctx, const float* sal, const float* mask, i64 nvox, int pass, uint32_t prefix,
                                uint64_t* hist_dev);
+enum : uint32_t { SELECT_NO_VOXEL = 1u, SELECT_INCONSISTENT = 2u };
+struct SelectState {
+  uint32_t prefix;
+  uint32_t flag;
+  uint64_t k;
+  uint64_t n;
+  float thr;
+  uint32_t pad;
+};
+struct StageReadback {
+  SelectState sel;
+  unsigned long long list_total;
+  unsigned list_flags, pad;
+};
+int dev_select_queue(visfd_hip_ctx* ctx, const float* sal, const float* mask, i64 nvox, float fraction, SelectState* state_dev);
+int select_result(const SelectState& s, float* thr_out);
+int select_rank_check(uint64_t n, float fraction);
 int dev_apply_threshold(visfd_hip_ctx* ctx, float* sal, i64 nvox, float thr);
 int dev_threshold_fraction(visfd_hip_ctx* ctx, float* sal, const float* mask, i64 nvox, float fraction,
                            float* thr_out);
diff --git a/visfd_amd/csrc/context.hip b/visfd_amd/csrc/context.hip
--- a/visfd_amd/csrc/context.hip
+++ b/visfd_amd/csrc/context.hip
@@ -64,6 +64,7 @@
 #define VH_OPT(field) {#field, &visfd_hip_options::field}
 const OptionDesc kOptions[] = {
     VH_OPT(gauss_3pass), VH_OPT(gauss_cfg), VH_OPT(gauss_wg_per_cu), VH_OPT(log_pair), VH_OPT(log_pair_chunk),
+    VH_OPT(membrane_queue),
     VH_OPT(tv_dense), VH_OPT(tv_fma), VH_OPT(gauss_fma), VH_OPT(eig_f32), VH_OPT(tv_zrun), VH_OPT(tv_no_replay),
     VH_OPT(tv_exact_tiled), VH_OPT(tv_no_fold), VH_OPT(tv_poison), VH_OPT(tv_reserve_wg), VH_OPT(tv_max_wg),
     VH_OPT(blob_test_cap), VH_OPT(morph_general), VH_OPT(morph_levels), VH_OPT(filter3d_general), VH_OPT(median_general),
@@ -184,6 +185,8 @@
   blob_jobs_abort(ctx);
   int rc = visfd_hip_trim(ctx);
   if (ctx->aux_stream) (void)hipStreamDestroy(ctx->aux_stream);
+  if (ctx->stage_event) (void)hipEventDestroy(ctx->stage_event);
+  if (ctx->stage_pinned) (void)hipHostFree(ctx->stage_pinned);
   if (ctx->own_stream) (void)hipStreamDestroy(ctx->stream);
   delete ctx;
   return rc;
diff --git a/visfd_amd/csrc/ridge.hip b/visfd_amd/csrc/ridge.hip
--- a/visfd_amd/csrc/ridge.hip
+++ b/visfd_amd/csrc/ridge.hip
@@ -152,7 +152,8 @@
 template <bool F32>
 __global__ void __launch_bounds__(BLOCK)
 ridge_directions_kernel(const float* __restrict__ S, const float* __restrict__ sal, int nx, int ny, int nz,
-                        float sigma, int order, float* __restrict__ dir) {
+                        float sigma, int order, float* __restrict__ dir,
+                        const float* __restrict__ thr_dev) {
   __shared__ unsigned short list[DIR_CHUNK];
   __shared__ int wave_tot[BLOCK / 64];
   const i64 nvox = (i64)nx * ny * nz;
@@ -160,10 +161,13 @@
   const int tid = threadIdx.x, lane = tid & 63, wave = tid >> 6;
   unsigned keep = 0u;
   int cnt = 0;
+  const bool cut = thr_dev != nullptr;
+  const float thr = cut ? *thr_dev : 0.0f;
 #pragma unroll
   for (int k = 0; k < DIR_PER; k++) {
     const i64 v = base + k * BLOCK + tid;
-    const bool kp = v < nvox && sal[v] != 0.0f;
+    const float sv = v < nvox ? sal[v] : 0.0f;
+    const bool kp = sv != 0.0f && !(cut && sv < thr);
     keep |= (kp ? 1u : 0u) << k;
     cnt += kp ? 1 : 0;
   }
@@ -324,13 +328,13 @@
 }
 
 int dev_ridge_directions(visfd_hip_ctx* ctx, const float* S, const float* sal, i64 nx, i64 ny, i64 nz, float sigma,
-                         int order, float* dir) {
+                         int order, float* dir, const float* thr_dev) {
   if (nx < 3 || ny < 3 || nz < 3)
     return fail(VISFD_HIP_EINVAL, "ridge detection requires an image at least 3 voxels wide in x,y,z");
   if (nx >= (1LL << 31) || ny >= (1LL << 31) || nz >= (1LL << 31)) return fail(VISFD_HIP_EINVAL, "dimension too large");
   const i64 nb = (nx * ny * nz + DIR_CHUNK - 1) / DIR_CHUNK;
   if (nb > 0x7fffffffLL) return fail(VISFD_HIP_EINVAL, "volume too large for one launch");
-  VH_EIG_LAUNCH(ridge_directions_kernel, dim3((unsigned)nb), S, sal, (int)nx, (int)ny, (int)nz, sigma, order, dir);
+  VH_EIG_LAUNCH(ridge_directions_kernel, dim3((unsigned)nb), S, sal, (int)nx, (int)ny, (int)nz, sigma, order, dir, thr_dev);
   VH_HIP(hipGetLastError());
   return VISFD_HIP_OK;
 }
diff --git a/visfd_amd/csrc/select.hip b/visfd_amd/csrc/select.hip
--- a/visfd_amd/csrc/select.hip
+++ b/visfd_amd/csrc/select.hip
@@ -2,6 +2,7 @@
 #include <vector>
 
 #include "common.hpp"
+#include "select_pick.hpp"
 
 namespace vh {
 
@@ -14,17 +15,19 @@
   const uint32_t u = __float_as_uint(f);
   return (u & 0x80000000u) ? ~u : (u | 0x80000000u);
 }
-inline float key_to_float(uint32_t k) {
+__host__ __device__ inline float key_to_float(uint32_t k) {
   const uint32_t u = (k & 0x80000000u) ? (k & 0x7fffffffu) : ~k;
   float f;
-  std::memcpy(&f, &u, 4);
+  __builtin_memcpy(&f, &u, 4);
   return f;
 }
 
+template <bool DEVPREFIX>
 __global__ void __launch_bounds__(BLOCK)
 histogram_kernel(const float* __restrict__ sal, const float* __restrict__ mask, i64 n, int round,
-                 uint32_t prefix, unsigned long long* __restrict__ hist) {
+                 uint32_t prefix_arg, const SelectState* __restrict__ state, unsigned long long* __restrict__ hist) {
   __shared__ unsigned int lh[NBINS];
+  const uint32_t prefix = DEVPREFIX ? state->prefix : prefix_arg;
   for (int i = threadIdx.x; i < NBINS; i += BLOCK) lh[i] = 0;
   __syncthreads();
   const int shift = (round == 0) ? 21 : (round == 1) ? 10 : 0;
@@ -60,6 +63,53 @@
 }
 
 __global__ void __launch_bounds__(BLOCK)
+pick_kernel(unsigned long long* __restrict__ hist, int round, float fraction, SelectState* __restrict__ state) {
+  constexpr int PER = NBINS / BLOCK;
+  __shared__ uint64_t lh[NBINS];
+  __shared__ uint64_t chunk[BLOCK];
+  const int t = threadIdx.x;
+  uint64_t sum = 0;
+#pragma unroll
+  for (int i = 0; i < PER; i++) {
+    const uint64_t c = hist[t * PER + i];
+    hist[t * PER + i] = 0;
+    lh[t * PER + i] = c;
+    sum += c;
+  }
+  chunk[t] = sum;
+  __syncthreads();
+  if (t != 0) return;
+  uint64_t k = 0;
+  uint32_t prefix = 0;
+  if (round == 0) {
+    uint64_t n = 0;
+    for (int i = 0; i < BLOCK; i++) n += chunk[i];
+    state->n = n;
+    state->flag = 0;
+    if (!select_rank(n, fraction, &k)) {
+      state->flag = SELECT_NO_VOXEL;
+      state->thr = __builtin_inff();
+      return;
+    }
+  } else {
+    if (state->flag) return;
+    k = state->k;
+    prefix = state->prefix;
+  }
+  const int c = select_pick_bin(chunk, BLOCK, &k);
+  const int d = c < 0 ? -1 : select_pick_bin(lh + c * PER, PER, &k);
+  if (d < 0) {
+    state->flag = SELECT_INCONSISTENT;
+    state->thr = __builtin_inff();
+    return;
+  }
+  prefix = (prefix << (round == 2 ? 10 : 11)) | (uint32_t)(c * PER + d);
+  state->prefix = prefix;
+  state->k = k;
+  if (round == 2) state->thr = key_to_float(prefix);
+}
+
+__global__ void __launch_bounds__(BLOCK)
 apply_threshold_kernel(float* __restrict__ sal, i64 n, float thr) {
   i64 i = (i64)blockIdx.x * BLOCK + threadIdx.x;
   const i64 step = (i64)gridDim.x * BLOCK;
@@ -78,7 +128,7 @@
   hipStream_t st = ctx->stream;
   VH_HIP(hipMemsetAsync(hist, 0, sizeof(unsigned long long) * NBINS, st));
   const unsigned g = grid_for(nvox, BLOCK, (i64)ctx->num_cus * 32);
-  histogram_kernel<<<dim3(g), dim3(BLOCK), 0, st>>>(sal, mask, nvox, pass, prefix, hist);
+  histogram_kernel<false><<<dim3(g), dim3(BLOCK), 0, st>>>(sal, mask, nvox, pass, prefix, nullptr, hist);
   VH_HIP(hipGetLastError());
   VH_HIP(hipMemcpyAsync(hist_host, hist, sizeof(uint64_t) * NBINS, hipMemcpyDeviceToHost, st));
   VH_HIP(hipStreamSynchronize(st));
@@ -95,7 +145,7 @@
   hipStream_t st = ctx->stream;
   VH_HIP(hipMemsetAsync(hist_dev, 0, sizeof(unsigned long long) * NBINS, st));
   const unsigned g = grid_for(nvox, BLOCK, (i64)ctx->num_cus * 32);
-  histogram_kernel<<<dim3(g), dim3(BLOCK), 0, st>>>(sal, mask, nvox, pass, prefix, reinterpret_cast<unsigned long long*>(hist_dev));
+  histogram_kernel<false><<<dim3(g), dim3(BLOCK), 0, st>>>(sal, mask, nvox, pass, prefix, nullptr, reinterpret_cast<unsigned long long*>(hist_dev));
   VH_HIP(hipGetLastError());
   return VISFD_HIP_OK;
 }
@@ -107,38 +157,63 @@
   return VISFD_HIP_OK;
 }
 
-static int pick_bin_descending(const std::vector<uint64_t>& h, uint64_t* k) {
-  uint64_t seen = 0;
-  for (int b = NBINS - 1; b >= 0; b--) {
-    if (seen + h[b] > *k) { *k -= seen; return b; }
-    seen += h[b];
-  }
-  return -1;
-}
-
-int select_pick_digit(const uint64_t* hist, uint64_t* k) {
-  return pick_bin_descending(std::vector<uint64_t>(hist, hist + NBINS), k);
-}
+int dev_select_queue(visfd_hip_ctx* ctx, const float* sal, const float* mask, i64 nvox, float fraction, SelectState* state) {
+  unsigned long long* hist = nullptr;
+  VH_TRY(ws(ctx, WS_HIST, (size_t)NBINS, &hist));
+  hipStream_t st = ctx->stream;
+  VH_HIP(hipMemsetAsync(hist, 0, sizeof(unsigned long long) * NBINS, st));
+  const unsigned g = grid_for(nvox, BLOCK, (i64)ctx->num_cus * 32);
+  for (int round = 0; round < 3; round++) {
+    histogram_kernel<true><<<dim3(g), dim3(BLOCK), 0, st>>>(sal, mask, nvox, round, 0u, state, hist);
+    pick_kernel<<<dim3(1), dim3(BLOCK), 0, st>>>(hist, round, fraction, state);
+  }
+  VH_HIP(hipGetLastError());
+  return VISFD_HIP_OK;
+}
+
+static const char* const kNoVoxel = "threshold fraction selects no voxel (the reference would read past its array)";
+static const char* const kInconsistent = "radix select: inconsistent histogram";
+
+int select_result(const SelectState& s, float* thr_out) {
+  if (s.flag & SELECT_NO_VOXEL) return fail(VISFD_HIP_EINVAL, kNoVoxel);
+  if (s.flag) return fail(VISFD_HIP_EDEVICE, kInconsistent);
+  if (thr_out) *thr_out = s.thr;
+  return VISFD_HIP_OK;
+}
+int select_rank_check(uint64_t n, float fraction) {
+  uint64_t k = 0;
+  if (!select_rank(n, fraction, &k)) return fail(VISFD_HIP_EINVAL, kNoVoxel);
+  return VISFD_HIP_OK;
+}
+
+int select_pick_digit(const uint64_t* hist, uint64_t* k) { return select_pick_bin(hist, NBINS, k); }
 float select_key_to_float(uint32_t key) { return key_to_float(key); }
 
 int dev_threshold_fraction(visfd_hip_ctx* ctx, float* sal, const float* mask, i64 nvox, float fraction,
                            float* thr_out) {
-  std::vector<uint64_t> h(NBINS);
-  uint64_t n_unmasked = 0;
-  VH_TRY(dev_select_histogram(ctx, sal, mask, nvox, 0, 0, h.data(), &n_unmasked));
-  const float prod = (float)n_unmasked * fraction;
-  uint64_t k = (uint64_t)std::floor(prod);
-  if (n_unmasked == 0 || k >= n_unmasked)
-    return fail(VISFD_HIP_EINVAL, "threshold fraction selects no voxel (the reference would read past its array)");
-  const int d0 = pick_bin_descending(h, &k);
-  if (d0 < 0) return fail(VISFD_HIP_EDEVICE, "radix select: inconsistent histogram");
-  VH_TRY(dev_select_histogram(ctx, sal, mask, nvox, 1, (uint32_t)d0, h.data(), nullptr));
-  const int d1 = pick_bin_descending(h, &k);
-  if (d1 < 0) return fail(VISFD_HIP_EDEVICE, "radix select: inconsistent histogram");
-  VH_TRY(dev_select_histogram(ctx, sal, mask, nvox, 2, ((uint32_t)d0 << 11) | (uint32_t)d1, h.data(), nullptr));
-  const int d2 = pick_bin_descending(h, &k);
-  if (d2 < 0) return fail(VISFD_HIP_EDEVICE, "radix select: inconsistent histogram");
-  const float thr = key_to_float(((uint32_t)d0 << 21) | ((uint32_t)d1 << 10) | (uint32_t)d2);
+  float thr = 0.0f;
+  if (ctx->opt.membrane_queue) {
+    StageReadback* block = nullptr;
+    VH_TRY(ws(ctx, WS_SELECT, 1, &block));
+    VH_TRY(dev_select_queue(ctx, sal, mask, nvox, fraction, &block->sel));
+    SelectState got;
+    VH_HIP(hipMemcpyAsync(&got, &block->sel, sizeof(got), hipMemcpyDeviceToHost, ctx->stream));
+    VH_HIP(hipStreamSynchronize(ctx->stream));
+    VH_TRY(select_result(got, &thr));
+  } else {
+    std::vector<uint64_t> h(NBINS);
+    uint64_t n_unmasked = 0, k = 0;
+    VH_TRY(dev_select_histogram(ctx, sal, mask, nvox, 0, 0, h.data(), &n_unmasked));
+    if (!select_rank(n_unmasked, fraction, &k)) return fail(VISFD_HIP_EINVAL, kNoVoxel);
+    uint32_t key = 0;
+    for (int round = 0; round < 3; round++) {
+      if (round > 0) VH_TRY(dev_select_histogram(ctx, sal, mask, nvox, round, key, h.data(), nullptr));
+      const int d = select_pick_bin(h.data(), NBINS, &k);
+      if (d < 0) return fail(VISFD_HIP_EDEVICE, kInconsistent);
+      key = (key << (round == 2 ? 10 : 11)) | (uint32_t)d;
+    }
+    thr = key_to_float(key);
+  }
   if (thr_out) *thr_out = thr;
   return dev_apply_threshold(ctx, sal, nvox, thr);
 }
diff --git a/visfd_amd/csrc/select_pick.hpp b/visfd_amd/csrc/select_pick.hpp
--- /dev/null
+++ b/visfd_amd/csrc/select_pick.hpp
@@ -0,0 +1,29 @@
+#pragma once
+
+#include <cmath>
+#include <cstdint>
+
+#if defined(__HIPCC__)
+#define VH_SELECT_HD __host__ __device__
+#else
+#define VH_SELECT_HD
+#endif
+
+namespace vh {
+
+VH_SELECT_HD inline bool select_rank(uint64_t n, float fraction, uint64_t* k) {
+  const float prod = (float)n * fraction;
+  *k = (uint64_t)floorf(prod);
+  return n != 0 && *k < n;
+}
+
+VH_SELECT_HD inline int select_pick_bin(const uint64_t* h, int nbins, uint64_t* k) {
+  uint64_t seen = 0;
+  for (int b = nbins - 1; b >= 0; b--) {
+    if (seen + h[b] > *k) { *k -= seen; return b; }
+    seen += h[b];
+  }
+  return -1;
+}
+
+}
diff --git a/visfd_amd/csrc/tv.hip b/visfd_amd/csrc/tv.hip
--- a/visfd_amd/csrc/tv.hip
+++ b/visfd_amd/csrc/tv.hip
@@ -207,6 +207,29 @@
                      cutoff);
 }
 
+int dev_tv_stage_count(visfd_hip_ctx* ctx, const float* sal, const float* thr_dev, const float* mask, i64 nx, i64 ny, i64 nz,
+                       float sigma_tv, int exponent, float cutoff, unsigned long long* total_dev, unsigned* flags_dev,
+                       TvStagePlan* plan) {
+  VH_TRY(check_dims(nx, ny, nz));
+  VH_TRY(check_dims32(nx, ny, nz));
+  const int h = host_tv_halfwidth(sigma_tv, cutoff);
+  VH_REQUIRE(h >= 0 && h <= 255, "tensor-voting window halfwidth out of range");
+  TvRoute routes[4];
+  tv_routes(ctx->opt, {sal, nullptr, nullptr, mask, mask, nx, ny, nz, 0, nz, exponent, false, false}, routes);
+  if (routes[0] != TvRoute::BoxTol && routes[0] != TvRoute::BoxExact) return TV_DECLINED;
+  TvTables tab;
+  VH_TRY(tv_table_device(ctx, sigma_tv, cutoff, h, &tab));
+  const bool exact = routes[0] == TvRoute::BoxExact;
+  *plan = {h, exact, exact ? tab.box_exact : tab.box_tol, tab.box_tol_sq, {}};
+  return dev_tv_box_count(ctx, sal, thr_dev, mask, nx, ny, nz, 0, nz, h, exponent, exact, total_dev, flags_dev, &plan->lists);
+}
+
+int dev_tv_stage_vote(visfd_hip_ctx* ctx, const TvStagePlan& plan, unsigned long long total, unsigned flags, const float* sal,
+                      const float* dir, float* ten, const float* mask, i64 nx, i64 ny, i64 nz, int exponent) {
+  return dev_tv_box_vote(ctx, plan.lists, total, flags, sal, dir, ten, mask, mask, nx, ny, nz, 0, nz, plan.h, plan.dtab_box,
+                         plan.dtab_box_sq, exponent, plan.exact);
+}
+
 int dev_tv_weight_sum(visfd_hip_ctx* ctx, const float* sal, float* den, const float* mask_src, const float* mask_dst, i64 nx,
                       i64 ny, i64 nz, float sigma_tv, float cutoff) {
   VH_TRY(check_dims(nx, ny, nz));
diff --git a/visfd_amd/csrc/tv_box.hip b/visfd_amd/csrc/tv_box.hip
--- a/visfd_amd/csrc/tv_box.hip
+++ b/visfd_amd/csrc/tv_box.hip
@@ -761,16 +761,16 @@
   return fold ? tv_box_kernel<2, true> : tv_box_kernel<2, false>;
 }
 
-}
-
-int dev_tv_box(visfd_hip_ctx* ctx, const float* sal, const float* dir, float* ten, const float* mask_src,
-               const float* mask_dst, i64 nx, i64 ny, i64 nz, i64 z_out0, i64 z_out1, int h, const float4* dtab_box,
-               const float4* dtab_box_sq, int exponent, bool exact) {
+struct BoxPlan {
+  BoxParams p;
+  size_t lds, lds_static;
+  i64 nblk;
+};
+int box_plan(visfd_hip_ctx* ctx, i64 nx, i64 ny, i64 nz, i64 z_out0, i64 z_out1, int h, int exponent, bool exact, BoxPlan* b) {
   if (exponent != 2 && exponent != 4) return TV_DECLINED;
   if (h < 1 || h > 40) return TV_DECLINED;
   if (nx * ny >= (1LL << 29) || nx > TV_LIST_MAX_NX || ny >= (1 << 24)) return TV_DECLINED;
-  hipStream_t st = ctx->stream;
-  BoxParams p;
+  BoxParams& p = b->p;
   p.nx = (int)nx; p.ny = (int)ny; p.nz = (int)nz;
   p.z_out0 = (int)z_out0; p.z_out1 = (int)z_out1;
   p.h = h;
@@ -782,19 +782,44 @@
   const size_t slice_bytes = sizeof(float4) * (size_t)p.nsl;
   p.tiles_x = (int)((nx + TX - 1) / TX);
   p.tiles_y = (int)((ny + TY - 1) / TY);
-  i64 nblk = 0;
-  VH_TRY(tv_plan_units(ctx, 8, p.tiles_x, p.tiles_y, z_out0, z_out1, &p.zrun, &nblk));
-  if (nblk == 0) return VISFD_HIP_OK;
-  const size_t lds = 2 * slice_bytes + sizeof(unsigned) * (size_t)(2 * h + 4) * NW * (exact ? NPAIR : 1);
-  const size_t lds_static = sizeof(float4) * (LSLOTS + 1) + sizeof(uint2) * LSLOTS + sizeof(uint2) * NW * NSUB * 2 * HCAP + 1536;
+  b->nblk = 0;
+  VH_TRY(tv_plan_units(ctx, 8, p.tiles_x, p.tiles_y, z_out0, z_out1, &p.zrun, &b->nblk));
+  b->lds = 2 * slice_bytes + sizeof(unsigned) * (size_t)(2 * h + 4) * NW * (exact ? NPAIR : 1);
+  b->lds_static = sizeof(float4) * (LSLOTS + 1) + sizeof(uint2) * LSLOTS + sizeof(uint2) * NW * NSUB * 2 * HCAP + 1536;
   static_assert(2 * HCAP == HX, "the two kernels' hit lists take the same LDS");
-  if (lds + lds_static > 150 * 1024) return TV_DECLINED;
-
+  if (b->nblk > 0 && b->lds + b->lds_static > 150 * 1024) return TV_DECLINED;
+  return VISFD_HIP_OK;
+}
+inline int list_mode(int exponent, bool exact) { return exact ? 1 : (exponent == 4 ? 0 : 2); }
+
+}
+
+int dev_tv_box_count(visfd_hip_ctx* ctx, const float* sal, const float* thr_dev, const float* mask_src, i64 nx, i64 ny, i64 nz,
+                     i64 z_out0, i64 z_out1, int h, int exponent, bool exact, unsigned long long* total_dev, unsigned* flags_dev,
+                     TvListPlan* plan) {
+  BoxPlan b;
+  VH_TRY(box_plan(ctx, nx, ny, nz, z_out0, z_out1, h, exponent, exact, &b));
+  if (b.nblk == 0) return TV_DECLINED;
+  unsigned* counter = nullptr;
+  VH_TRY(ws(ctx, WS_COUNTER, 16, &counter));
+  return tv_list_count(ctx, sal, thr_dev, mask_src, nx, ny, nz, z_out0, z_out1, h, list_mode(exponent, exact), counter, total_dev,
+                       flags_dev, plan);
+}
+
+int dev_tv_box_vote(visfd_hip_ctx* ctx, const TvListPlan& plan, unsigned long long total, unsigned flags, const float* sal,
+                    const float* dir, float* ten, const float* mask_src, const float* mask_dst, i64 nx, i64 ny, i64 nz, i64 z_out0,
+                    i64 z_out1, int h, const float4* dtab_box, const float4* dtab_box_sq, int exponent, bool exact) {
+  hipStream_t st = ctx->stream;
+  BoxPlan b;
+  VH_TRY(box_plan(ctx, nx, ny, nz, z_out0, z_out1, h, exponent, exact, &b));
+  BoxParams& p = b.p;
+  const size_t lds = b.lds, lds_static = b.lds_static;
+  const i64 nblk = b.nblk;
   unsigned* counter = nullptr;
   VH_TRY(ws(ctx, WS_COUNTER, 16, &counter));
   TvSenderLists L;
-  VH_TRY(tv_sender_lists(ctx, sal, dir, mask_src, nx, ny, nz, z_out0, z_out1, h, exact ? 1 : (exponent == 4 ? 0 : 2),
-                         exact ? (TVL_NON_FINITE | TVL_WEIGHTED_MASK) : 0u, !exact && !ctx->opt.tv_no_fold, counter, &L));
+  VH_TRY(tv_list_write(ctx, plan, sal, dir, mask_src, total, flags, exact ? (TVL_NON_FINITE | TVL_WEIGHTED_MASK) : 0u,
+                       !exact && !ctx->opt.tv_no_fold, &L));
   p.zl0 = L.zl0; p.nzl = L.nzl;
 
   size_t wg_per_cu = (160 * 1024) / (lds + lds_static);
@@ -836,4 +861,23 @@
   return VISFD_HIP_OK;
 }
 
-}
+int dev_tv_box(visfd_hip_ctx* ctx, const float* sal, const float* dir, float* ten, const float* mask_src,
+               const float* mask_dst, i64 nx, i64 ny, i64 nz, i64 z_out0, i64 z_out1, int h, const float4* dtab_box,
+               const float4* dtab_box_sq, int exponent, bool exact) {
+  BoxPlan b;
+  VH_TRY(box_plan(ctx, nx, ny, nz, z_out0, z_out1, h, exponent, exact, &b));
+  if (b.nblk == 0) return VISFD_HIP_OK;
+  unsigned* counter = nullptr;
+  VH_TRY(ws(ctx, WS_COUNTER, 16, &counter));
+  unsigned long long* const total_dev = reinterpret_cast<unsigned long long*>(counter + 4);
+  TvListPlan plan;
+  VH_TRY(tv_list_count(ctx, sal, nullptr, mask_src, nx, ny, nz, z_out0, z_out1, h, list_mode(exponent, exact), counter, total_dev,
+                       counter + 6, &plan));
+  unsigned long long tot2[2] = {0, 0};
+  VH_HIP(hipMemcpyAsync(tot2, total_dev, sizeof(tot2), hipMemcpyDeviceToHost, ctx->stream));
+  VH_HIP(hipStreamSynchronize(ctx->stream));
+  return dev_tv_box_vote(ctx, plan, tot2[0], (unsigned)tot2[1], sal, dir, ten, mask_src, mask_dst, nx, ny, nz, z_out0, z_out1, h,
+                         dtab_box, dtab_box_sq, exponent, exact);
+}
+
+}
diff --git a/visfd_amd/csrc/tv_common.hpp b/visfd_amd/csrc/tv_common.hpp
--- a/visfd_amd/csrc/tv_common.hpp
+++ b/visfd_amd/csrc/tv_common.hpp
@@ -102,8 +102,41 @@
   bool folded;
   int zl0, nzl;
 };
-int tv_sender_lists(visfd_hip_ctx* ctx, const float* sal, const float* dir, const float* mask_src, i64 nx, i64 ny, i64 nz,
-                    i64 z_out0, i64 z_out1, int h, int mode, unsigned decline_on, bool may_fold, unsigned* counter,
-                    TvSenderLists* out);
+struct TvListGeo {
+  int nx, ny, nz;
+  int zl0, nzl;
+  int ntx, h;
+};
+struct TvListPlan {
+  TvListGeo g;
+  unsigned* rows;
+  unsigned row_blocks;
+  int mode;
+  const float* thr_dev;
+};
+int tv_list_count(visfd_hip_ctx* ctx, const float* sal, const float* thr_dev, const float* mask_src, i64 nx, i64 ny, i64 nz,
+                  i64 z_out0, i64 z_out1, int h, int mode, unsigned* counter, unsigned long long* total_dev, unsigned* flags_dev,
+                  TvListPlan* plan);
+int tv_list_write(visfd_hip_ctx* ctx, const TvListPlan& plan, const float* sal, const float* dir, const float* mask_src,
+                  unsigned long long total, unsigned flags, unsigned decline_on, bool may_fold, TvSenderLists* out);
+
+int dev_tv_box_count(visfd_hip_ctx* ctx, const float* sal, const float* thr_dev, const float* mask_src, i64 nx, i64 ny, i64 nz,
+                     i64 z_out0, i64 z_out1, int h, int exponent, bool exact, unsigned long long* total_dev, unsigned* flags_dev,
+                     TvListPlan* plan);
+int dev_tv_box_vote(visfd_hip_ctx* ctx, const TvListPlan& plan, unsigned long long total, unsigned flags, const float* sal,
+                    const float* dir, float* ten, const float* mask_src, const float* mask_dst, i64 nx, i64 ny, i64 nz, i64 z_out0,
+                    i64 z_out1, int h, const float4* dtab_box, const float4* dtab_box_sq, int exponent, bool exact);
+
+struct TvStagePlan {
+  int h;
+  bool exact;
+  const float4 *dtab_box, *dtab_box_sq;
+  TvListPlan lists;
+};
+int dev_tv_stage_count(visfd_hip_ctx* ctx, const float* sal, const float* thr_dev, const float* mask, i64 nx, i64 ny, i64 nz,
+                       float sigma_tv, int exponent, float cutoff, unsigned long long* total_dev, unsigned* flags_dev,
+                       TvStagePlan* plan);
+int dev_tv_stage_vote(visfd_hip_ctx* ctx, const TvStagePlan& plan, unsigned long long total, unsigned flags, const float* sal,
+                      const float* dir, float* ten, const float* mask, i64 nx, i64 ny, i64 nz, int exponent);
 
 }
diff --git a/visfd_amd/csrc/tv_list.hip b/visfd_amd/csrc/tv_list.hip
--- a/visfd_amd/csrc/tv_list.hip
+++ b/visfd_amd/csrc/tv_list.hip
@@ -8,11 +8,7 @@
 
 namespace {
 
-struct ListGeo {
-  int nx, ny, nz;
-  int zl0, nzl;
-  int ntx, h;
-};
+using ListGeo = TvListGeo;
 constexpr int LNT = 256;
 constexpr int LWORDS_MAX = TV_LIST_MAX_NX / 32;
 
@@ -32,7 +28,8 @@
 tvl_row_kernel(const float* __restrict__ sal, const float* __restrict__ dir, const float* __restrict__ mask_src, ListGeo g,
                unsigned* __restrict__ rows, float4* __restrict__ ent, unsigned* __restrict__ pos,
                unsigned* __restrict__ neg_flag ,
-               int fold ) {
+               int fold ,
+               const float* __restrict__ thr_dev ) {
   constexpr int LB = 8;
   __shared__ unsigned bits_all[LNT / 64][LWORDS_MAX + 4];
   __shared__ unsigned base_all[WRITE ? LNT / 64 : 1][WRITE ? LWORDS_MAX * 2 + 4 : 1];
@@ -52,6 +49,8 @@
   }
   unsigned any = 0, total = 0;
   unsigned* const cum = cum_all[WRITE ? wave : 0];
+  const bool cut = thr_dev != nullptr;
+  const float thr = cut ? *thr_dev : 0.0f;
   for (int c0 = 0; c0 < nchunks; c0 += LB) {
     float v[LB], m[LB];
 #pragma unroll
@@ -63,7 +62,7 @@
 #pragma unroll
     for (int k = 0; k < LB; k++) {
       if (c0 + k >= nchunks) break;
-      const bool f = v[k] != 0.0f && m[k] != 0.0f;
+      const bool f = v[k] != 0.0f && m[k] != 0.0f && !(cut && v[k] < thr);
       const unsigned long long bal = __builtin_amdgcn_ballot_w64(f);
       if (lane == 0) {
         bits[2 * (c0 + k)] = (unsigned)bal;
@@ -150,9 +149,16 @@
 
 }
 
-int tv_sender_lists(visfd_hip_ctx* ctx, const float* sal, const float* dir, const float* mask_src, i64 nx, i64 ny, i64 nz,
-                    i64 z_out0, i64 z_out1, int h, int mode, unsigned decline_on, bool may_fold, unsigned* counter,
-                    TvSenderLists* out) {
+namespace {
+auto row_kernel(bool write, int mode) {
+  if (write) return mode == 1 ? tvl_row_kernel<true, 1> : mode == 0 ? tvl_row_kernel<true, 0> : tvl_row_kernel<true, 2>;
+  return mode == 1 ? tvl_row_kernel<false, 1> : mode == 0 ? tvl_row_kernel<false, 0> : tvl_row_kernel<false, 2>;
+}
+}
+
+int tv_list_count(visfd_hip_ctx* ctx, const float* sal, const float* thr_dev, const float* mask_src, i64 nx, i64 ny, i64 nz,
+                  i64 z_out0, i64 z_out1, int h, int mode, unsigned* counter, unsigned long long* total_dev, unsigned* flags_dev,
+                  TvListPlan* plan) {
   hipStream_t st = ctx->stream;
   ListGeo g;
   g.nx = (int)nx; g.ny = (int)ny; g.nz = (int)nz; g.h = h; g.ntx = (int)((nx + TX - 1) / TX);
@@ -162,20 +168,18 @@
   if ((i64)g.nzl * ny > 0x7fffffffLL) return TV_DECLINED;
   unsigned* rows = nullptr;
   if (ws(ctx, WS_TVLIST, nrows, &rows) != VISFD_HIP_OK) { set_error(""); (void)hipGetLastError(); return TV_DECLINED; }
-  unsigned long long* total_dev = reinterpret_cast<unsigned long long*>(counter + 4);
   VH_HIP(hipMemsetAsync(counter, 0, 16 * sizeof(unsigned), st));
   const unsigned row_blocks = (unsigned)(((i64)g.nzl * ny + LNT / 64 - 1) / (LNT / 64));
-  const auto row_pass = [&](auto kernel, float4* ent, unsigned* pos, int fold) {
-    kernel<<<dim3(row_blocks), dim3(LNT), 0, st>>>(sal, dir, mask_src, g, rows, ent, pos, counter + 6, fold);
-  };
-  row_pass(mode == 1 ? tvl_row_kernel<false, 1> : mode == 0 ? tvl_row_kernel<false, 0> : tvl_row_kernel<false, 2>, nullptr, nullptr, 0);
+  row_kernel(false, mode)<<<dim3(row_blocks), dim3(LNT), 0, st>>>(sal, nullptr, mask_src, g, rows, nullptr, nullptr, flags_dev, 0, thr_dev);
   tvl_scan_kernel<<<dim3((unsigned)(((size_t)g.nzl * g.ntx + LNT - 1) / LNT)), dim3(LNT), 0, st>>>(g, rows, total_dev);
   VH_HIP(hipGetLastError());
-  unsigned long long tot2[2] = {0, 0};
-  VH_HIP(hipMemcpyAsync(tot2, total_dev, sizeof(tot2), hipMemcpyDeviceToHost, st));
-  VH_HIP(hipStreamSynchronize(st));
-  const unsigned long long total = tot2[0];
-  const unsigned flags = (unsigned)tot2[1];
+  *plan = {g, rows, row_blocks, mode, thr_dev};
+  return VISFD_HIP_OK;
+}
+
+int tv_list_write(visfd_hip_ctx* ctx, const TvListPlan& plan, const float* sal, const float* dir, const float* mask_src,
+                  unsigned long long total, unsigned flags, unsigned decline_on, bool may_fold, TvSenderLists* out) {
+  hipStream_t st = ctx->stream;
   if (flags & decline_on) return TV_DECLINED;
   if (total >= (1ull << 32) - 2048) return TV_DECLINED;
   const int fold = (may_fold && !(flags & TVL_NOT_POSITIVE)) ? 1 : 0;
@@ -184,9 +188,10 @@
   float4* const ent = reinterpret_cast<float4*>(lists);
   unsigned* const pos = reinterpret_cast<unsigned*>(lists + (size_t)(total + 16) * 16);
   if (ctx->opt.tv_poison) VH_HIP(hipMemsetAsync(lists, 0xff, (size_t)(total + 16) * 20, st));
-  row_pass(mode == 1 ? tvl_row_kernel<true, 1> : mode == 0 ? tvl_row_kernel<true, 0> : tvl_row_kernel<true, 2>, ent, pos, fold);
+  row_kernel(true, plan.mode)<<<dim3(plan.row_blocks), dim3(LNT), 0, st>>>(sal, dir, mask_src, plan.g, plan.rows, ent, pos, nullptr, fold,
+                                                                           plan.thr_dev);
   VH_HIP(hipGetLastError());
-  *out = {ent, pos, rows, total, flags, fold != 0, g.zl0, g.nzl};
+  *out = {ent, pos, plan.rows, total, flags, fold != 0, plan.g.zl0, plan.g.nzl};
   return VISFD_HIP_OK;
 }
 
diff --git a/visfd_amd/pipeline.py b/visfd_amd/pipeline.py
--- a/visfd_amd/pipeline.py
+++ b/visfd_amd/pipeline.py
@@ -77,13 +77,18 @@
     bg = None
     if sigma_background > 0:
         bg = background if background is not None else src.new_empty(src.shape)
-        ctx.peak_background_dev(src, bg, sigma_background, ratio, mask)
-    ctx.ridge_scores_dev(src, sal, smoothed, sigma, ratio, order, mask, bg)
-    thr = ctx.threshold_fraction_dev(sal, best_fraction, mask)
-    ctx.ridge_directions_dev(smoothed, sal, dirs, sigma, order)
     sigma_tv = float(np.float32(tv_sigma_ratio) * np.float32(sigma))
-    ctx.tv_dense_stick_dev(sal, dirs, tensor, sigma_tv, tv_exponent, tv_truncate_ratio, mask, mask)
-    ctx.tensor_saliency_dev(tensor, sal, order, mask, src if bg is not None else None, bg)
+    if sigma_tv > 0:
+        thr = ctx.membrane_stage_dev(src, sal, dirs, tensor, smoothed, sigma, ratio, order, best_fraction, sigma_tv, tv_exponent,
+                                     tv_truncate_ratio, mask, sigma_background if bg is not None else 0.0, bg)
+    else:
+        if bg is not None:
+            ctx.peak_background_dev(src, bg, sigma_background, ratio, mask)
+        ctx.ridge_scores_dev(src, sal, smoothed, sigma, ratio, order, mask, bg)
+        thr = ctx.threshold_fraction_dev(sal, best_fraction, mask)
+        ctx.ridge_directions_dev(smoothed, sal, dirs, sigma, order)
+        ctx.tv_dense_stick_dev(sal, dirs, tensor, sigma_tv, tv_exponent, tv_truncate_ratio, mask, mask)
+        ctx.tensor_saliency_dev(tensor, sal, order, mask, src if bg is not None else None, bg)
     if tail is not None:
         if tail.get("map", api.MAP_NONE) not in (api.MAP_NONE, api.MAP_RESCALE):
             raise ValueError("membrane_detect: the threshold maps read the input image; only MAP_RESCALE acts on the saliency")
```
